# sunzeyeah/item-alignment

Measured on AMD Instinct MI355X. Metric: item-pairs/sec (train step) RoBERTa-large+ViT-B two-tower, higher is better.
Workload: dtype bf16

## Files before the change

include/itemalign.h:

```cpp
#ifndef ITEMALIGN_H
#define ITEMALIGN_H
#include <stddef.h>
#include <stdint.h>

#ifdef __cplusplus
extern "C" {
#endif

typedef struct ihipStream_t* ia_stream_t;

#define IA_OK 0
#define IA_ERR_ARG (-1)
#define IA_ERR_LAUNCH (-2)
#define IA_ERR_WORKSPACE (-3)
#define IA_ERR_UNSUPPORTED (-4)

const char* ia_strerror(int code);
#define IA_ABI_VERSION 20
int ia_abi_version(void);

#define IA_EPI_NONE 0
#define IA_EPI_BIAS 1
#define IA_EPI_BIAS_GELU 2
#define IA_EPI_ADD 3
// ... 10 lines not shown
size_t ia_gemm_colsum_workspace_bytes(int M, int N);
size_t ia_gemm_wgrad_rows_workspace_bytes(int N_out, int N_in, int M_rows);
int ia_gemm_wgrad_rows_filters(int N_out, int N_in, int M_rows);
int ia_gemm_wgrad_rows(const void* dY, int ldy, const void* X, int ldx, float* dW, int ldw, int N_out, int N_in, int M_rows,
                       const uint8_t* row_live, int accumulate, void* workspace, size_t workspace_bytes, ia_stream_t stream);
size_t ia_ktile_mask_bytes(int M_rows);
int ia_ktile_mask(const uint8_t* row_live, int M_rows, uint32_t* mask, ia_stream_t stream);
int ia_ktile_mask_host(const uint8_t* row_live, int M_rows, uint32_t* mask);
size_t ia_gemm_dgrad_rows_workspace_bytes(int M_rows, int N_in, int K_out);
int ia_gemm_dgrad_rows_filters(int M_rows, int N_in, int K_out);
int ia_gemm_dgrad_rows(const void* dY, int ldy, const void* W, int w_kstrided, int ldw, void* dX, int ldx, int M_rows, int N_in, int K_out,
                       int epilogue, const void* aux, int ldaux, void* C2, const uint8_t* row_live, void* workspace, size_t workspace_bytes,
                       ia_stream_t stream);
size_t ia_row_blocks_bytes(int M_rows);
int ia_row_blocks(const uint8_t* row_live, int M_rows, int* list, ia_stream_t stream);
int ia_row_blocks_host(const uint8_t* row_live, int M_rows, int* list);
int ia_debug_dgrad_rows(int on);
int ia_debug_fwd_rows(int on);
size_t ia_gemm_fwd_rows_workspace_bytes(int M_rows);
int ia_gemm_fwd_rows_filters(int M_rows, int N_out, int K_in);
int ia_gemm_fwd_rows(const void* X, int ldx, const void* W, int ldw, void* Y, int ldy, int M_rows, int N_out, int K_in, int epilogue,
                     const float* bias, void* C2, int scaled_cols, float col_scale, const uint8_t* row_live, int fill_dead_rows,
                     void* workspace, size_t workspace_bytes, ia_stream_t stream);
int ia_gemm_fwd_rows_add(const void* X, int ldx, const void* W, int ldw, void* Y, int ldy, int M_rows, int N_out, int K_in, const float* bias,
                         const void* aux, int ldaux, const uint8_t* row_live, int fill_dead_rows, void* workspace, size_t workspace_bytes,
                         ia_stream_t stream);
size_t ia_row_groups_bytes(int M_rows);
int ia_row_groups(const uint8_t* row_live, int M_rows, int* list, ia_stream_t stream);
int ia_row_groups_host(const uint8_t* row_live, int M_rows, int* list);
int ia_gemm_dgrad_groups_rows(const void* dY, int ldy, const void* W, int w_kstrided, int ldw, void* dX, int ldx, int M_rows, int N_in,
                              int K_out, const void* aux, int ldaux, void* C2, const uint8_t* row_live, void* workspace,
                              size_t workspace_bytes, ia_stream_t stream);
int ia_debug_out_rows(int on);

int ia_prof_begin(int variant, int max_launches);
int ia_prof_end(double* total_ms, double* total_flops, int* launches);
double ia_prof_bytes(void);
int ia_debug_cu_hog(int workgroups, float milliseconds, ia_stream_t stream);
int ia_debug_gemm_dynamic(int on);

int ia_ln_fwd(const void* x, const float* bias, const void* residual, void* z_out, void* y, float* mean, float* rstd,
              const float* gamma, const float* beta, int M, int H, float eps, float drop_p, uint32_t seed, uint32_t stream_id,
              ia_stream_t stream);
int ia_ln_fwd_rows(const void* x, const float* bias, const void* residual, void* z_out, void* y, float* mean, float* rstd,
                   const float* gamma, const float* beta, int M, int H, float eps, float drop_p, uint32_t seed, uint32_t stream_id,
                   const uint8_t* row_live, ia_stream_t stream);
size_t ia_ln_bwd_workspace_bytes(int M, int H);
int ia_ln_bwd(const void* dy, const void* dres, const void* z, const float* mean, const float* rstd, const float* gamma, void* dz,
              void* dx, float* dgamma, float* dbeta, float* dbias, int M, int H, float drop_p, uint32_t seed, uint32_t stream_id,
              void* workspace, size_t workspace_bytes, int accumulate, ia_stream_t stream);
int ia_ln_bwd2(const void* dy, const void* dy2, const void* dres, const void* z, const float* mean, const float* rstd, const float* gamma,
               void* dz, void* dx, float* dgamma, float* dbeta, float* dbias, int M, int H, float drop_p, uint32_t seed, uint32_t stream_id,
               void* workspace, size_t workspace_bytes, int accumulate, ia_stream_t stream);
int ia_ln_bwd2_rows(const void* dy, const void* dy2, const void* dres, const void* z, const float* mean, const float* rstd,
                    const float* gamma, void* dz, void* dx, float* dgamma, float* dbeta, float* dbias, int M, int H, float drop_p,
                    uint32_t seed, uint32_t stream_id, const uint8_t* row_live, void* workspace, size_t workspace_bytes, int accumulate,
                    ia_stream_t stream);
size_t ia_colsum_workspace_bytes(int M, int N);
int ia_colsum(const void* x, int ld, int M, int N, float* out, int accumulate, void* workspace, size_t workspace_bytes,
              ia_stream_t stream);

int ia_attn_fwd(const void* q, const void* k, const void* v, int ld_qkv, const uint8_t* key_mask, void* out, int ld_o, float* lse2,
                int B, int nh, int L, float scale, float drop_p, uint32_t seed, ia_stream_t stream);
int ia_attn_bwd(const void* q, const void* k, const void* v, int ld_qkv, const uint8_t* key_mask, const void* out, const void* d_out,
                int ld_o, const float* lse2, float* delta, void* dq, void* dk, void* dv, int ld_dqkv, int B, int nh, int L,
                float scale, float drop_p, uint32_t seed, ia_stream_t stream);
size_t ia_attn_bwd_bias_workspace_bytes(int B, int nh, int L);
int ia_attn_bwd_bias(const void* q, const void* k, const void* v, int ld_qkv, const uint8_t* key_mask, const void* out, const void* d_out,
                     int ld_o, const float* lse2, float* delta, void* dq, void* dk, void* dv, int ld_dqkv, float* dbias, void* workspace,
                     size_t workspace_bytes, int B, int nh, int L, float scale, float drop_p, uint32_t seed, ia_stream_t stream);

int ia_attn_fwd_ps(const void* q, const void* k, const void* v, int ld_qkv, const uint8_t* key_mask, void* out, int ld_o, float* lse2,
                   int B, int nh, int L, float scale, float drop_p, uint32_t seed, ia_stream_t stream);
int ia_attn_bwd_bias_ps(const void* q, const void* k, const void* v, int ld_qkv, const uint8_t* key_mask, const void* out, const void* d_out,
                        int ld_o, const float* lse2, float* delta, void* dq, void* dk, void* dv, int ld_dqkv, float* dbias, void* workspace,
                        size_t workspace_bytes, int B, int nh, int L, float scale, float drop_p, uint32_t seed, ia_stream_t stream);
#define IA_ATTN_Q_PRESCALED 1
#define IA_ATTN_MASKED_ROWS_DEAD 2
int ia_attn_bwd_bias_ex(int flags, const void* q, const void* k, const void* v, int ld_qkv, const uint8_t* key_mask, const void* out,
                        const void* d_out, int ld_o, const float* lse2, float* delta, void* dq, void* dk, void* dv, int ld_dqkv, float* dbias,
                        void* workspace, size_t workspace_bytes, int B, int nh, int L, float scale, float drop_p, uint32_t seed,
                        ia_stream_t stream);

int ia_attn_fwd_x(const void* q, int ld_q, const void* k, const void* v, int ld_kv, const uint8_t* key_mask, void* out, int ld_o,
                  float* lse2, int B, int nh, int Lq, int Lk, float scale, float drop_p, uint32_t seed, ia_stream_t stream);
int ia_attn_bwd_x(const void* q, int ld_q, const void* k, const void* v, int ld_kv, const uint8_t* key_mask, const void* out,
                  const void* d_out, int ld_o, const float* lse2, float* delta, void* dq, int ld_dq, void* dk, void* dv, int ld_dkv,
                  int B, int nh, int Lq, int Lk, float scale, float drop_p, uint32_t seed, ia_stream_t stream);
int ia_attn_fwd_causal_x(const void* q, int ld_q, const void* k, const void* v, int ld_kv, void* out, int ld_o, float* lse2, int B, int nh,
                         int Lk, int fold, float scale, ia_stream_t stream);
int ia_attn_bwd_causal_x(const void* q, int ld_q, const void* k, const void* v, int ld_kv, const void* out, const void* d_out, int ld_o,
                         const float* lse2, float* delta, void* dq, int ld_dq, void* dk, void* dv, int ld_dkv, int B, int nh, int Lk,
                         int fold, float scale, ia_stream_t stream);

int ia_rotary_split_fwd(const void* src, int ld_src, void* q_out, void* kv_out, int M, int n, int nh, ia_stream_t stream);
int ia_rotary_split_bwd(const void* dq, const void* dkv, void* dsrc, int ld_src, int M, int n, int nh, ia_stream_t stream);
int ia_swiglu_fwd(const void* src, int ld_src, void* out, int M, int F, ia_stream_t stream);
int ia_swiglu_bwd(const void* dout, const void* src, int ld_src, void* dsrc, int ld_dsrc, int M, int F, ia_stream_t stream);

int ia_kg_gather_fwd(const float* ent_table, const float* rel_table, const int64_t* ids, int ld_ids, int ent_col, int rel_lo,
                     float* h_sign, float* r, int B, int P, int Dk, ia_stream_t stream);
int ia_kg_gather_bwd(const float* dr, const int64_t* ids, int ld_ids, int rel_lo, float* rel_grad, int B, int P, int Dk,
                     ia_stream_t stream);
int ia_kg_rows_fwd(const float* h, const float* r, const float* hp, float* rows, int rows_per_item, int row0, int B, int P, int H,
                   ia_stream_t stream);
int ia_kg_rows_bwd(const float* drows, int rows_per_item, int row0, float* dh, float* dr, float* dhp, int B, int P, int H,
                   ia_stream_t stream);

#define IA_SIM_INNER 0
#define IA_SIM_COSINE 1
#define IA_SIM_L1 2
#define IA_SIM_L2 3
int ia_pair_sim_fwd(const float* x, const float* y, float* sim, float* probs, int B, int D, int measure, ia_stream_t stream);
int ia_pair_sim_bwd(const float* x, const float* y, const float* sim, const float* probs, const float* dsim, const float* dprobs,
                    float* dx, float* dy, int B, int D, int measure, ia_stream_t stream);
// ... 162 lines not shown
typedef struct {
  const void* w_qkv;
  const float* b_qkv;
  const void* w_o;
  const float* b_o;
  const float* ln1_g;
  const float* ln1_b;
  const void* w_fc1;
  const float* b_fc1;
  const void* w_fc2;
  const float* b_fc2;
  const float* ln2_g;
  const float* ln2_b;
  const void* wt_qkv;
  const void* wt_o;
  const void* wt_fc1;
  const void* wt_fc2;
} ia_layer_weights;

typedef struct {
  float* w_qkv; float* b_qkv; float* w_o; float* b_o; float* ln1_g; float* ln1_b;
  float* w_fc1; float* b_fc1; float* w_fc2; float* b_fc2; float* ln2_g; float* ln2_b;
} ia_layer_grads;

typedef struct {
  int B, L, H, I, nh;
  int pre_ln;
  float eps;
  float hidden_drop, attn_drop;
  uint32_t seed;
  uint32_t layer_id;
  const int* cu_seqlens;
  int total_tokens;
  float* dx_colsum_out;
  int dy_colsum_done;
  int masked_rows_dead;
  const int* row_blocks;
  const uint32_t* live_ktiles;
  const uint8_t* out_row_live;
  const int* out_row_blocks;
  const uint32_t* out_live_ktiles;
  const int* out_row_groups;
} ia_layer_cfg;

size_t ia_layer_stash_bytes(const ia_layer_cfg* cfg);
size_t ia_layer_bwd_scratch_bytes(const ia_layer_cfg* cfg);
int ia_layer_fwd(const ia_layer_cfg* cfg, const ia_layer_weights* w, const void* x, const uint8_t* key_mask, void* y, void* stash,
                 ia_stream_t stream);
size_t ia_layer_infer_scratch_bytes(const ia_layer_cfg* cfg);
int ia_layer_fwd_infer(const ia_layer_cfg* cfg, const ia_layer_weights* w, const void* x, const uint8_t* key_mask, void* y, void* scratch,
                       size_t scratch_bytes, ia_stream_t stream);
int ia_layer_bwd(const ia_layer_cfg* cfg, const ia_layer_weights* w, const ia_layer_grads* g, const void* x, const uint8_t* key_mask,
                 const void* y, const void* stash, const void* dy, void* dx, void* scratch, size_t scratch_bytes, ia_stream_t stream);
int ia_layer_bwd2(const ia_layer_cfg* cfg, const ia_layer_weights* w, const ia_layer_grads* g, const void* x, const uint8_t* key_mask,
                  const void* y, const void* stash, const void* dy, const void* dy2, void* dx, void* dx2, void* scratch,
                  size_t scratch_bytes, ia_stream_t stream);

#define IA_GCN_LONG_ROW 512
#define IA_GCN_SLAB_ROWS 1024
int ia_gcn_propagate_fwd(const int64_t* rowptr, const void* col, int col_is_64, const float* val, const float* x, const float* x0,
                         float* h, int N, int C, float alpha, float drop_p, uint32_t seed, uint32_t stream_id,
                         const int32_t* long_rows, int n_long, ia_stream_t stream);
int ia_gcn_propagate_bwd(const int64_t* rowptr_t, const void* col_t, int col_is_64, const float* val_t, const float* dh, float* dx,
                         float* dx0, int dx0_accumulate, int N, int C, float alpha, float drop_p, uint32_t seed, uint32_t stream_id,
                         const int32_t* long_rows_t, int n_long_t, ia_stream_t stream);
int ia_gcn_mix_fwd(const float* h, const float* W, float* out, int N, int C, float beta, float drop_p, uint32_t seed, uint32_t stream_id,
// ... 39 lines not shown
```

item_alignment_amd/_lib.py:

```python
import ctypes as C
import os

_HERE = os.path.dirname(os.path.abspath(__file__))
LIB_PATH = os.path.join(_HERE, "libitemalign_hip.so")

vp, i32, u32, f32, sz = C.c_void_p, C.c_int, C.c_uint32, C.c_float, C.c_size_t
PP, IP = C.POINTER(C.c_void_p), C.POINTER(C.c_int)


class LayerWeights(C.Structure):
    _fields_ = [(n, vp) for n in ("w_qkv", "b_qkv", "w_o", "b_o", "ln1_g", "ln1_b", "w_fc1", "b_fc1", "w_fc2", "b_fc2",
                                  "ln2_g", "ln2_b", "wt_qkv", "wt_o", "wt_fc1", "wt_fc2")]


class LayerGrads(C.Structure):
    _fields_ = [(n, vp) for n in ("w_qkv", "b_qkv", "w_o", "b_o", "ln1_g", "ln1_b", "w_fc1", "b_fc1", "w_fc2", "b_fc2",
                                  "ln2_g", "ln2_b")]


class LayerCfg(C.Structure):
    _fields_ = [("B", i32), ("L", i32), ("H", i32), ("I", i32), ("nh", i32), ("pre_ln", i32), ("eps", f32),
                ("hidden_drop", f32), ("attn_drop", f32), ("seed", u32), ("layer_id", u32), ("cu_seqlens", vp), ("total_tokens", i32),
                ("dx_colsum_out", vp), ("dy_colsum_done", i32), ("masked_rows_dead", i32),
                ("row_blocks", vp), ("live_ktiles", vp),
                ("out_row_live", vp), ("out_row_blocks", vp), ("out_live_ktiles", vp), ("out_row_groups", vp)]


SIGNATURES = {
    "ia_strerror": (C.c_char_p, [i32]),
    "ia_abi_version": (i32, []),
    "ia_gemm_bf16": (i32, [vp, i32, i32, vp, i32, i32, vp, i32, i32, i32, i32, i32, i32, vp, vp, i32, vp, i32, vp, sz, vp]),
    "ia_gemm_workspace_bytes": (sz, [i32, i32, i32, i32]),
    "ia_gemm_colsum_workspace_bytes": (sz, [i32, i32]),
    "ia_gemm_wgrad_rows_workspace_bytes": (sz, [i32, i32, i32]),
    "ia_gemm_wgrad_rows_filters": (i32, [i32, i32, i32]),
    "ia_gemm_wgrad_rows": (i32, [vp, i32, vp, i32, vp, i32, i32, i32, i32, vp, i32, vp, sz, vp]),
    "ia_ktile_mask_bytes": (sz, [i32]),
    "ia_ktile_mask": (i32, [vp, i32, vp, vp]),
    "ia_ktile_mask_host": (i32, [vp, i32, vp]),
    "ia_gemm_dgrad_rows_workspace_bytes": (sz, [i32, i32, i32]),
    "ia_gemm_dgrad_rows_filters": (i32, [i32, i32, i32]),
    "ia_gemm_dgrad_rows": (i32, [vp, i32, vp, i32, i32, vp, i32, i32, i32, i32, i32, vp, i32, vp, vp, vp, sz, vp]),
    "ia_row_blocks_bytes": (sz, [i32]),
    "ia_row_blocks": (i32, [vp, i32, vp, vp]),
    "ia_row_blocks_host": (i32, [vp, i32, vp]),
    "ia_debug_dgrad_rows": (i32, [i32]),
    "ia_gemm_fwd_rows_workspace_bytes": (sz, [i32]),
    "ia_gemm_fwd_rows_filters": (i32, [i32, i32, i32]),
    "ia_gemm_fwd_rows": (i32, [vp, i32, vp, i32, vp, i32, i32, i32, i32, i32, vp, vp, i32, f32, vp, i32, vp, sz, vp]),
    "ia_debug_fwd_rows": (i32, [i32]),
    "ia_gemm_fwd_rows_add": (i32, [vp, i32, vp, i32, vp, i32, i32, i32, i32, vp, vp, i32, vp, i32, vp, sz, vp]),
    "ia_row_groups_bytes": (sz, [i32]),
    "ia_row_groups": (i32, [vp, i32, vp, vp]),
    "ia_row_groups_host": (i32, [vp, i32, vp]),
    "ia_gemm_dgrad_groups_rows": (i32, [vp, i32, vp, i32, i32, vp, i32, i32, i32, i32, vp, i32, vp, vp, vp, sz, vp]),
    "ia_debug_out_rows": (i32, [i32]),
    "ia_prof_begin": (i32, [i32, i32]),
    "ia_prof_end": (i32, [C.POINTER(C.c_double), C.POINTER(C.c_double), C.POINTER(i32)]),
    "ia_prof_bytes": (C.c_double, []),
    "ia_debug_cu_hog": (i32, [i32, C.c_float, vp]),
    "ia_debug_gemm_dynamic": (i32, [i32]),
    "ia_ln_fwd": (i32, [vp, vp, vp, vp, vp, vp, vp, vp, vp, i32, i32, f32, f32, u32, u32, vp]),
    "ia_ln_fwd_rows": (i32, [vp, vp, vp, vp, vp, vp, vp, vp, vp, i32, i32, f32, f32, u32, u32, vp, vp]),
    "ia_ln_bwd_workspace_bytes": (sz, [i32, i32]),
    "ia_ln_bwd": (i32, [vp, vp, vp, vp, vp, vp, vp, vp, vp, vp, vp, i32, i32, f32, u32, u32, vp, sz, i32, vp]),
    "ia_ln_bwd2": (i32, [vp, vp, vp, vp, vp, vp, vp, vp, vp, vp, vp, vp, i32, i32, f32, u32, u32, vp, sz, i32, vp]),
    "ia_ln_bwd2_rows": (i32, [vp, vp, vp, vp, vp, vp, vp, vp, vp, vp, vp, vp, i32, i32, f32, u32, u32, vp, vp, sz, i32, vp]),
    "ia_colsum_workspace_bytes": (sz, [i32, i32]),
    "ia_colsum": (i32, [vp, i32, i32, i32, vp, i32, vp, sz, vp]),
    "ia_attn_fwd": (i32, [vp, vp, vp, i32, vp, vp, i32, vp, i32, i32, i32, f32, f32, u32, vp]),
    "ia_attn_bwd": (i32, [vp, vp, vp, i32, vp, vp, vp, i32, vp, vp, vp, vp, vp, i32, i32, i32, i32, f32, f32, u32, vp]),
    "ia_attn_bwd_bias_workspace_bytes": (sz, [i32, i32, i32]),
    "ia_attn_bwd_bias": (i32, [vp, vp, vp, i32, vp, vp, vp, i32, vp, vp, vp, vp, vp, i32, vp, vp, sz, i32, i32, i32, f32, f32, u32, vp]),
    "ia_attn_fwd_ps": (i32, [vp, vp, vp, i32, vp, vp, i32, vp, i32, i32, i32, f32, f32, u32, vp]),
    "ia_attn_bwd_bias_ps": (i32, [vp, vp, vp, i32, vp, vp, vp, i32, vp, vp, vp, vp, vp, i32, vp, vp, sz, i32, i32, i32, f32, f32, u32, vp]),
    "ia_attn_bwd_bias_ex": (i32, [i32, vp, vp, vp, i32, vp, vp, vp, i32, vp, vp, vp, vp, vp, i32, vp, vp, sz, i32, i32, i32, f32, f32, u32, vp]),
    "ia_gemm_bf16_qscale": (i32, [vp, i32, vp, i32, vp, i32, i32, i32, i32, vp, i32, f32, vp]),
    "ia_attn_fwd_x": (i32, [vp, i32, vp, vp, i32, vp, vp, i32, vp, i32, i32, i32, i32, f32, f32, u32, vp]),
    "ia_attn_bwd_x": (i32, [vp, i32, vp, vp, i32, vp, vp, vp, i32, vp, vp, vp, i32, vp, vp, i32, i32, i32, i32, i32, f32, f32, u32, vp]),
    "ia_attn_fwd_causal_x": (i32, [vp, i32, vp, vp, i32, vp, i32, vp, i32, i32, i32, i32, f32, vp]),
    "ia_attn_bwd_causal_x": (i32, [vp, i32, vp, vp, i32, vp, vp, i32, vp, vp, vp, i32, vp, vp, i32, i32, i32, i32, i32, f32, vp]),
    "ia_rotary_split_fwd": (i32, [vp, i32, vp, vp, i32, i32, i32, vp]),
    "ia_rotary_split_bwd": (i32, [vp, vp, vp, i32, i32, i32, i32, vp]),
    "ia_swiglu_fwd": (i32, [vp, i32, vp, i32, i32, vp]),
    "ia_swiglu_bwd": (i32, [vp, vp, i32, vp, i32, i32, i32, vp]),
    "ia_kg_gather_fwd": (i32, [vp, vp, vp, i32, i32, i32, vp, vp, i32, i32, i32, vp]),
    "ia_kg_gather_bwd": (i32, [vp, vp, i32, i32, vp, i32, i32, i32, vp]),
    "ia_kg_rows_fwd": (i32, [vp, vp, vp, vp, i32, i32, i32, i32, i32, vp]),
    "ia_kg_rows_bwd": (i32, [vp, i32, i32, vp, vp, vp, i32, i32, i32, vp]),
    "ia_pair_sim_fwd": (i32, [vp, vp, vp, vp, i32, i32, i32, vp]),
    "ia_pair_sim_bwd": (i32, [vp, vp, vp, vp, vp, vp, vp, vp, i32, i32, i32, vp]),
    "ia_nchw_to_nhwc_bf16": (i32, [vp, vp, i32, i32, i32, i32, i32, vp]),
    "ia_conv_nhwc_workspace_bytes": (sz, [i32, i32, i32, i32, i32, i32, i32, i32]),
    "ia_conv_nhwc_fwd": (i32, [vp, vp, vp, vp, i32, i32, i32, i32, i32, i32, i32, i32, vp, sz, vp]),
    "ia_conv_nhwc_bwd_data": (i32, [vp, vp, vp, i32, i32, i32, i32, i32, i32, i32, i32, vp, sz, vp]),
    "ia_conv_nhwc_bwd_weight": (i32, [vp, vp, vp, vp, i32, i32, i32, i32, i32, i32, i32, i32, i32, vp, sz, vp]),
    "ia_ws_conv_weight_fwd": (i32, [vp, vp, vp, vp, vp, i32, i32, i32, i32, f32, f32, vp]),
    "ia_ws_conv_weight_bwd": (i32, [vp, vp, vp, vp, vp, vp, vp, i32, i32, i32, i32, f32, vp]),
    "ia_silu_fwd": (i32, [vp, vp, sz, f32, vp]),
    "ia_silu_bwd": (i32, [vp, vp, vp, vp, sz, f32, vp]),
    "ia_silu_bwd_sum": (i32, [vp, vp, vp, vp, vp, sz, f32, vp]),
    "ia_avgpool2_fwd": (i32, [vp, vp, i32, i32, i32, i32, vp]),
    "ia_avgpool2_bwd": (i32, [vp, vp, i32, i32, i32, i32, vp]),
    "ia_gap_workspace_bytes": (sz, [i32, i32, i32]),
    "ia_gap_fwd": (i32, [vp, vp, i32, i32, i32, vp, sz, vp]),
    "ia_gap_bwd": (i32, [vp, vp, i32, i32, i32, vp]),
    "ia_eca_fwd": (i32, [vp, vp, i32, vp, vp, vp, vp, i32, i32, i32, f32, vp, sz, vp]),
    "ia_eca_fwd_linear_workspace_bytes": (sz, [i32, i32, i32]),
    "ia_eca_fwd_linear": (i32, [vp, vp, vp, vp, i32, vp, i32, vp, vp, vp, f32, vp, vp, i32, i32, i32, f32, vp, sz, vp]),
# ... 140 lines not shown
```

item_alignment_amd/csrc/attention.hip:

```cpp
#include "common.h"
#include <type_traits>
#include <cstdlib>

#define IA_ATTN_Q_PRESCALED 1
#define IA_ATTN_MASKED_ROWS_DEAD 2
extern "C" size_t ia_attn_bwd_bias_workspace_bytes(int B, int nh, int L);

namespace {

constexpr uint32_t OOB = 0xFFFFFFF0u;
constexpr float LOG2E = 1.4426950408889634f;

struct AttnArgs {
  const bf16* q; const bf16* k; const bf16* v;
  const bf16* o; const bf16* d_o;
  bf16* out;
  bf16* dq; bf16* dk; bf16* dv;
  const uint8_t* mask;
  float* lse2;
  float* delta;
  int B, nh, Lq, Lk;
  const int* cu;
  int ld_q, ld_kv, ld_o, ld_dq, ld_dkv;
  uint32_t q_bytes, kv_bytes, o_bytes;
  float sc;
  float scale;
  int q_prescaled;
  uint32_t thr16; float inv_keep; uint32_t seed;
  float* cs_part;
  int exact_delta;
  int dead_queries;
};

IA_DEV void attn_block_coords(const AttnArgs& p, int nt, int& tile, int& h, int& b) {
  const int nwg = gridDim.x, bid = blockIdx.x;
  const int per = nwg >> 3, r = nwg & 7, xcd = bid & 7, idx = bid >> 3;
  int w = (xcd < r ? xcd * (per + 1) : r * (per + 1) + (xcd - r) * per) + idx;
  tile = w % nt; w /= nt;
  h = w % p.nh; b = w / p.nh;
}

constexpr int MAX_KT = 32;
IA_DEV void build_valid_table(const AttnArgs& p, uint32_t (*s_valid)[2], size_t rowbase, int L, int lane, int wave) {
  const int nkt = (L + 63) >> 6;
  for (int t = wave; t < nkt; t += 4) {
    const int key = t * 64 + lane;
    const bool kv = key < L && (p.mask == nullptr || p.mask[rowbase + key] != 0);
    const uint64_t vb = __ballot(kv);
    if (lane == 0) { s_valid[t][0] = (uint32_t)vb; s_valid[t][1] = (uint32_t)(vb >> 32); }
  }
}

IA_DEV int swz_b128(int row) { return (row >> 1) & 7; }
IA_DEV int swz_tr(int row) { return ((row >> 1) & 1) << 2; }

IA_DEV void stage_rows32(__amdgpu_buffer_rsrc_t rs, char* slot, size_t row0, int nvalid, int ld, int col0, int lane) {
#pragma unroll
  for (int i = 0; i < 4; ++i) {
    const int row = i * 8 + (lane >> 3);
    const int c = (lane & 7) ^ swz_b128(row);
    uint32_t off = (uint32_t)(((row0 + row) * ld + col0 + c * 8) * 2);
    if (row >= nvalid) off = OOB;
    __builtin_amdgcn_raw_ptr_buffer_load_lds(rs, IA_LDS(slot + i * 1024), 16, off, 0, 0, 0);
  }
// ... 53 lines not shown
    *reinterpret_cast<bf16x4*>(w + 64 + rg * 16) = c;
  }
  asm volatile("s_waitcnt lgkmcnt(0)" ::: "memory");
  float cs[8];
#pragma unroll
  for (int j = 0; j < 8; ++j) cs[j] = 0.f;
#pragma unroll
  for (int i = 0; i < 4; ++i) {
    const int row = i * 8 + (lane >> 3), c = lane & 7;
    const bf16x8 v = *reinterpret_cast<const bf16x8*>(slot + row * EPI_ROW + c * 16);
    if (row < nrows) {
      *reinterpret_cast<bf16x8*>(out + (size_t)row * ld + c * 8) = v;
      if (cs_out) {
#pragma unroll
        for (int j = 0; j < 8; ++j) cs[j] += bf2f(v[j]);
      }
    }
  }
  if (cs_out) {
#pragma unroll
    for (int j = 0; j < 8; ++j) {
      float x = cs[j];
      x += ia_dpp<0x128>(x);
      cs[j] = ia_add_xor32(ia_add_xor16(x));
    }
    if (lane < 8) {
      *reinterpret_cast<f32x4*>(cs_out + lane * 8) = f32x4{cs[0], cs[1], cs[2], cs[3]};
      *reinterpret_cast<f32x4*>(cs_out + lane * 8 + 4) = f32x4{cs[4], cs[5], cs[6], cs[7]};
    }
  }
}
IA_DEV void zero_cs_row(float* cs_out, int lane) {
  if (lane < 16) *reinterpret_cast<f32x4*>(cs_out + lane * 4) = f32x4{0.f, 0.f, 0.f, 0.f};
}

namespace fwd3 {
constexpr int k_slot(int s) { return s == 2 ? 32768 : s * 8192; }
constexpr int v_slot(int s) { return s == 2 ? 40960 : 16384 + s * 8192; }
constexpr int Q_OFF = 32768, EPI_OFF = 0, TAB_OFF = 49152, SMEM = TAB_OFF + MAX_KT * 8;
constexpr uint32_t L_LO_BITS = 0x0D800000u, L_HI_BITS = 0x5D800000u;
constexpr float NEG_BIG = -1e30f;
constexpr uint32_t NEG_BIG_BF16 = 0xF14Au;

template <int OFF>
IA_DEV bf16x8 lds_read_b128(uint32_t addr) {
  bf16x8 d;
  asm volatile("ds_read_b128 %0, %1 offset:%2" : "=v"(d) : "v"(addr), "n"(OFF));
  return d;
}
template <int N>
IA_DEV void frag_wait(bf16x8 (&f)[8]) {
  asm volatile("s_waitcnt lgkmcnt(%8)" : "+v"(f[0]), "+v"(f[1]), "+v"(f[2]), "+v"(f[3]), "+v"(f[4]), "+v"(f[5]), "+v"(f[6]), "+v"(f[7]) : "n"(N));
}
IA_DEV float swap32(float x) {
  float a = x, b = x;
  asm volatile("s_nop 1\n\tv_permlane32_swap_b32 %0, %1\n\ts_nop 1" : "+v"(a), "+v"(b));
  return (threadIdx.x & 32) ? a : b;
}
IA_DEV f32x16 mfma(bf16x8 a, bf16x8 b, f32x16 c) { return __builtin_amdgcn_mfma_f32_32x32x16_bf16(a, b, c, 0, 0, 0); }

struct Lane {
  uint32_t ka[4];
  uint32_t v0, v1;
  uint32_t dk0, dk1, dv0, dv1;
};

// ... 78 lines not shown
  row.l_run *= alpha;
#pragma unroll
  for (int r = 0; r < 16; ++r) {
    s[r] = __builtin_amdgcn_exp2f(s[r] - m_new);
    o0[r] *= alpha; o1[r] *= alpha;
  }
  if (other) {
#pragma unroll
    for (int r = 0; r < 16; ++r) (*other)[r] += shift;
  }
}
}

template <bool DROPOUT, int QB>
__global__ __launch_bounds__(256, QB == 1 ? 3 : 2) void attn_fwd3_kernel(AttnArgs p) {
  using namespace fwd3;
  constexpr int ROWS = 128 * QB;
  constexpr int QX_OFF = SMEM;
  __shared__ __attribute__((aligned(16))) char smem[SMEM + (QB - 1) * 16384];
  uint32_t (*s_valid)[2] = reinterpret_cast<uint32_t (*)[2]>(smem + TAB_OFF);
  const int tid = threadIdx.x, lane = tid & 63, hh = lane >> 5, lq = lane & 31;
  const int wave = __builtin_amdgcn_readfirstlane(tid >> 6);
  int tile, h, b;
  attn_block_coords(p, (p.Lq + ROWS - 1) / ROWS, tile, h, b);
  int Lq = p.Lq, L = p.Lk;
  size_t qbase = (size_t)b * Lq, rowbase = (size_t)b * L;
  if (p.cu) {
    const int c0 = p.cu[b];
    Lq = L = p.cu[b + 1] - c0;
    qbase = rowbase = (size_t)c0;
    if (tile * ROWS >= Lq) return;
  }
  const int q0 = tile * ROWS + wave * 32 * QB;
  const bool active = q0 < Lq;
  const uint32_t win = (uint32_t)(((size_t)(L - 1) * p.ld_kv + 64) * 2);
  const __amdgpu_buffer_rsrc_t rsK = ia_rsrc(p.k + rowbase * p.ld_kv + h * 64, win);
  const __amdgpu_buffer_rsrc_t rsV = ia_rsrc(p.v + rowbase * p.ld_kv + h * 64, win);
  const uint32_t sbase = lds_addr(smem);
  const uint32_t tile_bytes = (uint32_t)p.ld_kv * 128u;
  const int nkt_all = (L + 63) >> 6;

  Lane ln;
  {
    const uint32_t a0 = (uint32_t)(lq * 128 + ((hh ^ swz_b128(lq)) << 4));
#pragma unroll
    for (int kb = 0; kb < 4; ++kb) ln.ka[kb] = sbase + (a0 ^ (uint32_t)(kb << 5));
    ln.v0 = sbase + tr_lane_off(lane, 0); ln.v1 = sbase + tr_lane_off(lane, 32);
    const int r0 = tid >> 3, r1 = 32 + (tid >> 3), c = tid & 7;
    ln.dk0 = (uint32_t)((r0 * p.ld_kv + (c ^ swz_b128(r0)) * 8) * 2); ln.dk1 = (uint32_t)((r1 * p.ld_kv + (c ^ swz_b128(r1)) * 8) * 2);
    ln.dv0 = (uint32_t)((r0 * p.ld_kv + (c ^ swz_tr(r0)) * 8) * 2);   ln.dv1 = (uint32_t)((r1 * p.ld_kv + (c ^ swz_tr(r1)) * 8) * 2);
  }
  typedef __attribute__((address_space(3))) char lds_char;
  lds_char* const lsm = (lds_char*)IA_LDS(smem);
  auto stage_k = [&](auto SLOT_T, int kt) {
    constexpr int S = decltype(SLOT_T)::value;
    const uint32_t so = (uint32_t)kt * tile_bytes;
    __builtin_amdgcn_raw_ptr_buffer_load_lds(rsK, (lsm + k_slot(S) + wave * 1024), 16, ln.dk0, so, 0, 0);
    __builtin_amdgcn_raw_ptr_buffer_load_lds(rsK, (lsm + k_slot(S) + 4096 + wave * 1024), 16, ln.dk1, so, 0, 0);
  };
  auto stage_v = [&](auto SLOT_T, int kt) {
    constexpr int S = decltype(SLOT_T)::value;
    const uint32_t so = (uint32_t)kt * tile_bytes;
    __builtin_amdgcn_raw_ptr_buffer_load_lds(rsV, (lsm + v_slot(S) + wave * 1024), 16, ln.dv0, so, 0, 0);
    __builtin_amdgcn_raw_ptr_buffer_load_lds(rsV, (lsm + v_slot(S) + 4096 + wave * 1024), 16, ln.dv1, so, 0, 0);
  };
  using S0 = std::integral_constant<int, 0>; using S1 = std::integral_constant<int, 1>; using S2 = std::integral_constant<int, 2>;

// ... 236 lines not shown
  for (int kb = 0; kb < 4; ++kb) {
    const bf16x8 raw = frag_b128(rq, lq, kb * 2 + hh);
    gf[kb] = frag_b128(rg, lq, kb * 2 + hh);
    const bf16x8 ov = frag_b128(ro, lq, kb * 2 + hh);
#pragma unroll
    for (int j = 0; j < 8; ++j) {
      dlt += bf2f(ov[j]) * bf2f(gf[kb][j]);
      qf[kb][j] = !p.q_prescaled ? f2bf(bf2f(raw[j]) * p.sc) : raw[j];
    }
  }
  dlt += swap32(dlt);
  if (p.exact_delta) dlt = p.delta[sidx];
  else if (active && hh == 0 && q < Lq) p.delta[sidx] = dlt;
  f32x16 nl, nd;
#pragma unroll
  for (int r = 0; r < 16; ++r) { nl[r] = -lse; nd[r] = DROPOUT ? 0.f : -dlt; }
  asm volatile("s_waitcnt lgkmcnt(0)" ::: "memory");
  __builtin_amdgcn_s_barrier();
  int nkt = nkt_all;
  uint32_t ragged = 0u;
  for (int t = 0; t < nkt_all; ++t) {
    const uint32_t lo = s_valid[t][0], hi = s_valid[t][1];
    if ((lo & hi) != 0xFFFFFFFFu) ragged |= 1u << t;
    if ((lo | hi) != 0u) nkt = t + 1;
  }
  bool work = active;
  if (p.dead_queries && p.cu == nullptr && p.Lq == p.Lk) {
    const uint32_t mine = active ? s_valid[q0 >> 6][(q0 >> 5) & 1] : 0u;
    const int t128 = tile * 2;
    uint32_t any = s_valid[t128][0] | s_valid[t128][1];
    if (t128 + 1 < nkt_all) any |= s_valid[t128 + 1][0] | s_valid[t128 + 1][1];
    work = active && __builtin_amdgcn_readfirstlane(mine) != 0u;
    if (__builtin_amdgcn_readfirstlane(any) == 0u) nkt = 1;
  }
  nkt = __builtin_amdgcn_readfirstlane(nkt);
  ragged = __builtin_amdgcn_readfirstlane(ragged);
  if (nkt > 1) stage_tile(S1{}, 1);
  const uint32_t rk = DROPOUT ? ia_rng_row(p.seed, (uint32_t)(b * p.nh + h), (uint32_t)q) : 0u;
  const uint32_t thr1 = DROPOUT ? (p.thr16 - 1u) * 0x10001u : 0u;
  f32x16 dq0 = zero16(), dq1 = zero16();

  auto tile_step = [&](auto SLOT_T, int t) {
    constexpr int SB = decltype(SLOT_T)::value * STAGE;
    using NEXT2 = std::integral_constant<int, (decltype(SLOT_T)::value + 2) % 3>;
    const bool LAST = t + 1 >= nkt;
    if (LAST) asm volatile("s_waitcnt vmcnt(0)" ::: "memory");
    else asm volatile("s_waitcnt vmcnt(4)" ::: "memory");
    __builtin_amdgcn_s_barrier();
    if (t + 2 < nkt) stage_tile(NEXT2{}, t + 2);
    if (!work) return;
    bf16x8 xk0, xk1, xv0, xv1, yk0, yk1, yv0, yv1;
    auto rd = [&](auto KB, bf16x8& k0, bf16x8& k1, bf16x8& v0, bf16x8& v1) {
      constexpr int kb = decltype(KB)::value;
      k0 = lds_read_b128<SB>(ka[kb]); k1 = lds_read_b128<SB + 4096>(ka[kb]);
      v0 = lds_read_b128<SB + 8192>(ka[kb]); v1 = lds_read_b128<SB + 12288>(ka[kb]);
    };
    using I0 = std::integral_constant<int, 0>; using I1 = std::integral_constant<int, 1>;
    using I2 = std::integral_constant<int, 2>; using I3 = std::integral_constant<int, 3>;
    rd(I0{}, xk0, xk1, xv0, xv1);
    rd(I1{}, yk0, yk1, yv0, yv1);
    f32x16 s0, s1, dp0, dp1;
    const bool plain = !((ragged >> t) & 1u);
    frag_wait4<4>(xk0, xk1, xv0, xv1);
    s0 = mfma(xk0, qf[0], nl); s1 = mfma(xk1, qf[0], nl);
    dp0 = mfma(xv0, gf[0], nd); dp1 = mfma(xv1, gf[0], nd);
    if (!plain) {
// ... 313 lines not shown
#pragma unroll
    for (int j = 0; j < 8; ++j) { kf[kb][j] = f2bf(-bf2f(kr[j])); vf[kb][j] = f2bf(-bf2f(vr[j])); }
  }
  const bool scale_q = !p.q_prescaled;
  if (scale_q) {
#pragma unroll
    for (int i = 0; i < 2; ++i) {
      bf16x8* const qp = reinterpret_cast<bf16x8*>(smem + i * 4096 + wave * 1024 + lane * 16);
      bf16x8 v = *qp;
#pragma unroll
      for (int j = 0; j < 8; ++j) v[j] = f2bf(bf2f(v[j]) * p.sc);
      *qp = v;
    }
  }
  int* const s_last = reinterpret_cast<int*>(smem + 3 * KV_STAGE + 1024 + 512);
  const bool trim = p.dead_queries && p.mask != nullptr && p.cu == nullptr && p.Lq == p.Lk;
  if (trim) {
    int last = -1;
    for (int base = wave * 64; base < Lq; base += 256) {
      const int pos = base + lane;
      const bool ok = pos < Lq && p.mask[rowbase + pos] != 0;
      const uint64_t bal = __ballot(ok);
      if (bal) last = base + 63 - __builtin_clzll(bal);
    }
    if (lane == 0) s_last[wave] = last;
  }
  asm volatile("s_waitcnt lgkmcnt(0)" ::: "memory");
  __builtin_amdgcn_s_barrier();
  if (trim) {
    const int last = max(max(s_last[0], s_last[1]), max(s_last[2], s_last[3]));
    const int live = __builtin_amdgcn_readfirstlane(last < 0 ? 1 : (last >> 6) + 1);
    if (live < nqt) nqt = live;
  }
  if (nqt > 1) stage_tile(S1{}, 1);
  f32x16 dk0 = zero16(), dk1 = zero16(), dv0 = zero16(), dv1 = zero16();

  auto prescale = [&](int stage_base) {
#pragma unroll
    for (int i = 0; i < 2; ++i) {
      bf16x8* const qp = reinterpret_cast<bf16x8*>(smem + stage_base + i * 4096 + wave * 1024 + lane * 16);
      bf16x8 v = *qp;
#pragma unroll
      for (int j = 0; j < 8; ++j) v[j] = f2bf(bf2f(v[j]) * sc);
      *qp = v;
    }
  };
  auto tile_step = [&](auto SLOT_T, int qt) {
    constexpr int SB = decltype(SLOT_T)::value * KV_STAGE;
    using NEXT2 = std::integral_constant<int, (decltype(SLOT_T)::value + 2) % 3>;
    if (qt + 1 >= nqt) asm volatile("s_waitcnt vmcnt(0)" ::: "memory");
    else asm volatile("s_waitcnt vmcnt(5)" ::: "memory");
    asm volatile("s_waitcnt lgkmcnt(0)" ::: "memory");
    __builtin_amdgcn_s_barrier();
    if (qt + 2 < nqt) stage_tile(NEXT2{}, qt + 2);
    if (!active) {
      if (scale_q && qt + 1 < nqt) {
        if (qt + 2 < nqt) asm volatile("s_waitcnt vmcnt(5)" ::: "memory");
        else asm volatile("s_waitcnt vmcnt(0)" ::: "memory");
        prescale(((decltype(SLOT_T)::value + 1) % 3) * KV_STAGE);
      }
      return;
    }
    if (DROPOUT) {
      s_rk[lane] = ia_rng_row(seed, stream_id, (uint32_t)(qt * 64 + lane));
      __builtin_amdgcn_wave_barrier();
    }
// ... 36 lines not shown
        for (int rg = 0; rg < 4; ++rg) rkq[rg] = *(const lds_u32x4*)(s_rk + qs * 32 + 8 * rg + 4 * hh);
      }
#pragma unroll
      for (int r = 0; r < 16; ++r) {
        const float pv = __builtin_amdgcn_exp2f(-s[r]);
        float pd = pv, nds;
        if (DROPOUT) {
          const uint32_t hsh = ia_rng_pair(rkq[r >> 2][r & 3], pc);
          const uint32_t dr = (hsh >> ush) & 0xFFFFu;
          const float mk = __builtin_fminf(__builtin_fmaxf((float)((int)dr - (int)thr1), 0.f), 1.f);
          pd = pv * mk;
          nds = pv * __builtin_fmaf(dp[r] * mk, inv_keep, dlr[r]);
        } else {
          nds = pv * dp[r];
        }
        pf[r >> 3][r & 7] = f2bf(pd);
        sf[r >> 3][r & 7] = f2bf(nds);
      }
      tr_wait<12>(g0);
      dv0 = mfma(g0.a0(), pf[0], dv0); dv1 = mfma(g0.a1(), pf[0], dv1);
      tr_wait<8>(a0);
      dk0 = mfma(a0.a0(), sf[0], dk0); dk1 = mfma(a0.a1(), sf[0], dk1);
      tr_wait<4>(g1);
      dv0 = mfma(g1.a0(), pf[1], dv0); dv1 = mfma(g1.a1(), pf[1], dv1);
      tr_wait<0>(a1);
      dk0 = mfma(a1.a0(), sf[1], dk0); dk1 = mfma(a1.a1(), sf[1], dk1);
    };
    sub_tile(std::integral_constant<int, 0>{});
    if (scale_q && qt + 1 < nqt) {
      if (qt + 2 < nqt) asm volatile("s_waitcnt vmcnt(5)" ::: "memory");
      else asm volatile("s_waitcnt vmcnt(0)" ::: "memory");
      prescale(((decltype(SLOT_T)::value + 1) % 3) * KV_STAGE);
    }
    if (qt * 64 + 32 < Lq) sub_tile(std::integral_constant<int, 1>{});
  };
  {
    int qt = 0;
    for (;;) {
      tile_step(S0{}, qt); if (++qt >= nqt) break;
      tile_step(S1{}, qt); if (++qt >= nqt) break;
      tile_step(S2{}, qt); if (++qt >= nqt) break;
    }
  }
  __builtin_amdgcn_s_barrier();
  float* cs_lds = p.cs_part ? reinterpret_cast<float*>(smem + 8 * EPI_SLOT) + wave * 128 : nullptr;
  if (!active && !cs_lds) return;
  if (active) {
    store_block_rows(smem + wave * 2 * EPI_SLOT, dk0, dk1, -1.f / LOG2E, !key_ok, p.dk + (rowbase + k0) * p.ld_dkv + h * 64, p.ld_dkv,
                     L - k0, lane, cs_lds);
    store_block_rows(smem + (wave * 2 + 1) * EPI_SLOT, dv0, dv1, DROPOUT ? p.inv_keep : 1.f, !key_ok, p.dv + (rowbase + k0) * p.ld_dkv + h * 64,
                     p.ld_dkv, L - k0, lane, cs_lds ? cs_lds + 64 : nullptr);
  } else { zero_cs_row(cs_lds, lane); zero_cs_row(cs_lds + 64, lane); }
  if (cs_lds) {
    __syncthreads();
    if (wave < 2) {
      const float* c = reinterpret_cast<const float*>(smem + 8 * EPI_SLOT) + wave * 64;
      p.cs_part[(size_t)(b * ((p.Lk + 127) >> 7) + tile) * (3 * p.nh * 64) + (1 + wave) * p.nh * 64 + h * 64 + lane] =
          (c[lane] + c[128 + lane]) + (c[256 + lane] + c[384 + lane]);
    }
  }
}

namespace bwdf {
using namespace bwd3;
constexpr int NW = 8, RING = 4;
constexpr int SL_Q = 0, SL_G = 4096, SL_O = 8192, SL_LSE = 12288, SL_DLT = SL_LSE + 256, SL_RK = SL_LSE + 384, SLOT = SL_LSE + 512;
constexpr int DLT_F = (SL_DLT - SL_LSE) / 4;
// ... 113 lines not shown
      for (int i = 0; i < 8; ++i) d += bf2f(gv[i]) * bf2f(ov[i]);
      d += ia_dpp<0xB1>(d); d += ia_dpp<0x4E>(d); d += ia_dpp<0x141>(d);
      if (c8 == 0) *reinterpret_cast<float*>(sl + SL_DLT + ((wave - 4) * 8 + r8) * 4) = d;
    }
  };

  const uint32_t thr1 = DROPOUT ? p.thr16 - 1u : 0u;
  const float inv_keep = p.inv_keep;
  const int ntile = (L + 127) >> 7;

  Cur prod{first_item, first_item / nh, first_item % nh};
  Cur cons = prod, kvn = prod;
  int pj = 0;
  issue_kv(kvn); adv(kvn);
#pragma unroll 1
  for (int s = 0; s < RING; ++s) {
    issue_ring(prod, pj, s);
    if (++pj == nb) { pj = 0; adv(prod); }
  }
  asm volatile("s_waitcnt vmcnt(0)" ::: "memory");
  prep(cons.it, 0, 0);
  asm volatile("s_waitcnt lgkmcnt(0)" ::: "memory");
  __builtin_amdgcn_s_barrier();

  bf16x8 kf[4], vf[4], KT[8];
  f32x16 dk0, dk1, dv0, dv1;
  f32x4 csq;
  bool key_ok = false, mine = false;
  uint32_t vbits = 0u;
  float pen = 0.f;
  bool any_bad = false;
  uint32_t pc = 0u, ush = 0u;
  const int G = cnt * nb;
  int cj = 0;
  Cur prev = cons;
  int pcj = 0;
#pragma unroll 1
  for (int g = 0;; ++g) {
    const bool haveA = g < G;
    const bool first = cj == 0, last = cj == nb - 1;
    auto part_a = [&](int ga, bool first_a, int blk) {
      {
        const int slot = ga & (RING - 1), par = ga & 1;
        if (first_a) {
          const char* kb_ = smem + KST + wave * 4096;
          const char* vb_ = smem + VST + wave * 4096;
#pragma unroll
          for (int kb = 0; kb < 4; ++kb) {
            const bf16x8 kr = frag_u(kb_, lk, kb * 2 + hh), vr = frag_u(vb_, lk, kb * 2 + hh);
#pragma unroll
            for (int i = 0; i < 8; ++i) { kf[kb][i] = f2bf(-bf2f(kr[i])); vf[kb][i] = f2bf(-bf2f(vr[i])); }
          }
          {
            s16x4 lo[8], hi[8];
#pragma unroll
            for (int k = 0; k < 8; ++k) { lo[k] = tr_read<0>(ktb + k * 4096); hi[k] = tr_read<2048>(ktb + k * 4096); }
            asm volatile("s_waitcnt lgkmcnt(0)" : "+v"(lo[0]), "+v"(lo[1]), "+v"(lo[2]), "+v"(lo[3]), "+v"(lo[4]), "+v"(lo[5]), "+v"(lo[6]), "+v"(lo[7]));
            asm volatile("" : "+v"(hi[0]), "+v"(hi[1]), "+v"(hi[2]), "+v"(hi[3]), "+v"(hi[4]), "+v"(hi[5]), "+v"(hi[6]), "+v"(hi[7]));
#pragma unroll
            for (int k = 0; k < 8; ++k) KT[k] = join(lo[k], hi[k]);
          }
          const int key = wave * 32 + lk;
          {
            const uint32_t* const mw = reinterpret_cast<const uint32_t*>(smem + MSK_OFF);
            uint32_t vb = 0u;
#pragma unroll
            for (int k = 0; k < 8; ++k) vb |= (mw[k] != 0u ? 1u : 0u) << k;
            vbits = __builtin_amdgcn_readfirstlane(vb);
            key_ok = ((mw[wave] >> lk) & 1u) != 0u;
          }
          mine = ((vbits >> wave) & 1u) != 0u;
          pen = key_ok ? 0.f : PEN;
          any_bad = __ballot(!key_ok) != 0ull;
          pc = pair_c_of(key); ush = (uint32_t)(key & 1) * 16u;
          dk0 = zero16(); dk1 = zero16(); dv0 = zero16(); dv1 = zero16();
          csq = f32x4{0.f, 0.f, 0.f, 0.f};
        }
        if (mine && (!p.dead_queries || ((vbits >> blk) & 1u))) {
          const uint32_t so = (uint32_t)(slot * SLOT);
          f32x16 s, dp;
          const float* const sL = reinterpret_cast<const float*>(smem + RING_OFF + slot * SLOT + SL_LSE) + 4 * hh;
          {
#pragma unroll
            for (int rg = 0; rg < 4; ++rg) {
              const f32x4 ls = *reinterpret_cast<const f32x4*>(sL + 8 * rg);
              const f32x4 dl = *reinterpret_cast<const f32x4*>(sL + DLT_F + 8 * rg);
#pragma unroll
              for (int j = 0; j < 4; ++j) { s[rg * 4 + j] = ls[j]; dp[rg * 4 + j] = DROPOUT ? 0.f : dl[j]; }
            }
            if (any_bad) {
#pragma unroll
              for (int r = 0; r < 16; ++r) s[r] += pen;
            }
          }
          const uint32_t k0_ = ka0 + so;
          bf16x8 xq, xg, yq, yg;
          xq = lds_read_b128<SL_Q>(k0_); xg = lds_read_b128<SL_G>(k0_);
          yq = lds_read_b128<SL_Q>(k0_ ^ 32u); yg = lds_read_b128<SL_G>(k0_ ^ 32u);
          asm volatile("s_waitcnt lgkmcnt(2)" : "+v"(xq), "+v"(xg));
          s = mfma(xq, kf[0], s); dp = mfma(xg, vf[0], dp);
          xq = lds_read_b128<SL_Q>(k0_ ^ 64u); xg = lds_read_b128<SL_G>(k0_ ^ 64u);
          asm volatile("s_waitcnt lgkmcnt(2)" : "+v"(yq), "+v"(yg));
          s = mfma(yq, kf[1], s); dp = mfma(yg, vf[1], dp);
          yq = lds_read_b128<SL_Q>(k0_ ^ 96u); yg = lds_read_b128<SL_G>(k0_ ^ 96u);
          asm volatile("s_waitcnt lgkmcnt(2)" : "+v"(xq), "+v"(xg));
          s = mfma(xq, kf[2], s); dp = mfma(xg, vf[2], dp);
          const uint32_t a0_ = t0 + so, a1_ = a0_ + t1d, a0x = a0_ ^ 32u, a1x = a1_ ^ 32u;
          TrPair g0, q0, g1, q1;
          read_tr<SL_G, 0>(g0, a0_, a1_, a0x, a1x);
          read_tr<SL_Q, 0>(q0, a0_, a1_, a0x, a1x);
          asm volatile("s_waitcnt lgkmcnt(8)" : "+v"(yq), "+v"(yg));
// ... 19 lines not shown
              pf[hf][rr] = f2bf(pd);
              sf[hf][rr] = f2bf(nds);
            }
            const int xa = xwo + par * XT;
            *reinterpret_cast<bf16x4*>(smem + (xa ^ (hf * 32))) = bf16x4{sf[hf][0], sf[hf][1], sf[hf][2], sf[hf][3]};
            *reinterpret_cast<bf16x4*>(smem + (xa ^ (hf * 32 + 16))) = bf16x4{sf[hf][4], sf[hf][5], sf[hf][6], sf[hf][7]};
          };
          half(std::integral_constant<int, 0>{});
          read_tr<SL_G, 16>(g1, a0_, a1_, a0x, a1x);
          read_tr<SL_Q, 16>(q1, a0_, a1_, a0x, a1x);
          tr_wait<12>(g0);
          dv0 = mfma(g0.a0(), pf[0], dv0); dv1 = mfma(g0.a1(), pf[0], dv1);
          tr_wait<8>(q0);
          dk0 = mfma(q0.a0(), sf[0], dk0); dk1 = mfma(q0.a1(), sf[0], dk1);
          half(std::integral_constant<int, 1>{});
          tr_wait<4>(g1);
          dv0 = mfma(g1.a0(), pf[1], dv0); dv1 = mfma(g1.a1(), pf[1], dv1);
          tr_wait<0>(q1);
          dk0 = mfma(q1.a0(), sf[1], dk0); dk1 = mfma(q1.a1(), sf[1], dk1);
        }
      }
    };
    auto part_c = [&]() {
      if (haveA && g >= 1) {
        if (cj == 1) { issue_kv(kvn); adv(kvn); }
        issue_ring(prod, pj, (g - 1) & (RING - 1));
        if (++pj == nb) { pj = 0; adv(prod); }
      }
      if (g == 0) return;
      {
        const uint32_t xr = xrb + ((g - 1) & 1) * XT, xr2 = xr ^ 16u;
        s16x4 lo[8], hi[8];
        f32x4 acc = {0.f, 0.f, 0.f, 0.f};
        if (!p.dead_queries || ((vbits >> pcj) & 1u)) {
#pragma unroll
        for (int k = 0; k < 8; ++k) { lo[k] = tr_read<0>(xr + k * 2 * XT); hi[k] = tr_read<16 * XP>(xr2 + k * 2 * XT); }
#define IA_DQ_STEP(k, n)                                                                                   \
        wait2<n>(lo[k], hi[k]);                                                                            \
        if ((vbits >> k) & 1u) acc = mfma16(KT[k], join(lo[k], hi[k]), acc);
        IA_DQ_STEP(0, 14) IA_DQ_STEP(1, 12) IA_DQ_STEP(2, 10) IA_DQ_STEP(3, 8) IA_DQ_STEP(4, 6) IA_DQ_STEP(5, 4) IA_DQ_STEP(6, 2) IA_DQ_STEP(7, 0)
#undef IA_DQ_STEP
        }
        const int q = pcj * 32 + 16 * qh + p16;
        bf16x4 o4;
#pragma unroll
        for (int i = 0; i < 4; ++i) { o4[i] = f2bf(-p.scale * acc[i]); }
        if (q < L) {
          *reinterpret_cast<bf16x4*>(p.dq + ((size_t)prev.b * L + q) * p.ld_dq + prev.h * 64 + 16 * dqt + 4 * g4) = o4;
#pragma unroll
          for (int i = 0; i < 4; ++i) csq[i] += bf2f(o4[i]);
        }
      }
      if (!first) return;
      asm volatile("s_waitcnt lgkmcnt(0)" ::: "memory");
      __builtin_amdgcn_s_barrier();
      const size_t row0 = (size_t)prev.b * L;
      float* const cs_w = reinterpret_cast<float*>(smem + CS_OFF) + wave * 128;
      if (wave < nb) {
        store_block_rows(smem + X_OFF + wave * EPI_SLOT, dk0, dk1, -1.f / LOG2E, false, p.dk + (row0 + wave * 32) * p.ld_dkv + prev.h * 64, p.ld_dkv,
                         L - wave * 32, lane, p.cs_part ? cs_w : nullptr);
        store_block_rows(smem + X_OFF + wave * EPI_SLOT, dv0, dv1, DROPOUT ? inv_keep : 1.f, false, p.dv + (row0 + wave * 32) * p.ld_dkv + prev.h * 64,
                         p.ld_dkv, L - wave * 32, lane, p.cs_part ? cs_w + 64 : nullptr);
      } else if (p.cs_part) { zero_cs_row(cs_w, lane); zero_cs_row(cs_w + 64, lane); }
      if (p.cs_part) {
        int ln = lane;
        asm volatile("" : "+v"(ln));
        float* const cq = reinterpret_cast<float*>(smem + CS_OFF + NW * 128 * 4);
// ... 67 lines not shown
  a.inv_keep = drop_p > 0.f ? 1.f / (1.f - (float)a.thr16 / 65536.f) : 1.f;
  a.seed = seed;
  return IA_OK;
}

bool exact_delta_on() { const char* e = getenv("IA_ATTN_EXACT_DELTA"); return e && atoi(e) != 0; }
bool fused_applies(const AttnArgs& a) {
  return !a.exact_delta && a.cu == nullptr && a.Lq == a.Lk && a.Lq > 32 && a.Lq <= 256 && a.delta != nullptr;
}
template <bool D> void launch_fused(const AttnArgs& a, hipStream_t st) {
  hipLaunchKernelGGL(attn_key_bits_kernel, dim3(a.B), dim3(64), 0, st, a.mask, reinterpret_cast<uint32_t*>(a.delta), a.Lk);
  const int per_x = (a.B * a.nh + 7) / 8;
  const dim3 grid(8 * (per_x < 32 ? per_x : 32));
  hipLaunchKernelGGL(attn_bwd_fused_kernel<D>, grid, dim3(512), 0, st, a);
}
template <bool D> void launch_pair(const AttnArgs& a, hipStream_t st) {
  const dim3 gq(((a.Lq + 127) / 128) * a.nh * a.B), gk(((a.Lk + 127) / 128) * a.nh * a.B), blk(256);
  if (a.exact_delta) hipLaunchKernelGGL(attn_bwd3_delta_kernel<D>, gq, blk, 0, st, a);
  hipLaunchKernelGGL(attn_bwd3_dq_kernel<D>, gq, blk, 0, st, a);
  hipLaunchKernelGGL(attn_bwd3_dkv_kernel<D>, gk, blk, 0, st, a);
}
template <bool D> void launch_bwd(const AttnArgs& a, hipStream_t st) {
  if (fused_applies(a)) launch_fused<D>(a, st);
  else launch_pair<D>(a, st);
}
template <bool D> void launch_fwd(const AttnArgs& a, hipStream_t st) {
  if (((a.Lq - 1) & 255) < 128) hipLaunchKernelGGL((attn_fwd3_kernel<D, 1>), dim3(((a.Lq + 127) / 128) * a.nh * a.B), dim3(256), 0, st, a);
  else hipLaunchKernelGGL((attn_fwd3_kernel<D, 2>), dim3(((a.Lq + 255) / 256) * a.nh * a.B), dim3(256), 0, st, a);
}

struct Packed { const int* cu; int total; };
struct BiasOut { float* dbias; void* workspace; size_t workspace_bytes; };

int attn_fwd_impl(int flags, const void* q, int ld_q, const void* k, const void* v, int ld_kv, const uint8_t* key_mask, const Packed* pk, void* out,
                  int ld_o, float* lse2, int B, int nh, int Lq, int Lk, float scale, float drop_p, uint32_t seed, hipStream_t stream) {
  (void)hipGetLastError();
  if (!q || !k || !v || !out || (pk && (!pk->cu || pk->total <= 0))) return IA_ERR_ARG;
  AttnArgs a{};
  const int rc = fill_args(a, B, nh, Lq, Lk, ld_q, ld_kv, ld_o, scale, drop_p, seed, pk ? pk->total : 0);
  if (rc) return rc;
  a.q = (const bf16*)q; a.k = (const bf16*)k; a.v = (const bf16*)v; a.out = (bf16*)out; a.mask = key_mask; a.lse2 = lse2;
  a.cu = pk ? pk->cu : nullptr;
  a.q_prescaled = (flags & IA_ATTN_Q_PRESCALED) ? 1 : 0;
  if (a.thr16) launch_fwd<true>(a, stream);
  else launch_fwd<false>(a, stream);
  return ia_check_launch();
}

int attn_bwd_impl(int flags, const void* q, int ld_q, const void* k, const void* v, int ld_kv, const uint8_t* key_mask, const Packed* pk,
                  const void* out, const void* d_out, int ld_o, const float* lse2, float* delta, void* dq, int ld_dq, void* dk, void* dv, int ld_dkv,
                  const BiasOut* bias, int B, int nh, int Lq, int Lk, float scale, float drop_p, uint32_t seed, hipStream_t stream) {
  (void)hipGetLastError();
  if (!q || !k || !v || !out || !d_out || !lse2 || !delta || !dq || !dk || !dv) return IA_ERR_ARG;
  if ((pk && (!pk->cu || pk->total <= 0)) || (bias && !bias->dbias)) return IA_ERR_ARG;
  if (bias && (!bias->workspace || bias->workspace_bytes < ia_attn_bwd_bias_workspace_bytes(B, nh, Lq))) return IA_ERR_WORKSPACE;
  AttnArgs a{};
  int rc = fill_args(a, B, nh, Lq, Lk, ld_q, ld_kv, ld_o, scale, drop_p, seed, pk ? pk->total : 0);
  if (rc) return rc;
  if ((ld_dq & 7) || (ld_dkv & 7) || ld_dq < nh * 64 || ld_dkv < nh * 64) return IA_ERR_ARG;
  a.q = (const bf16*)q; a.k = (const bf16*)k; a.v = (const bf16*)v; a.o = (const bf16*)out; a.d_o = (const bf16*)d_out;
  a.mask = key_mask; a.lse2 = const_cast<float*>(lse2); a.delta = delta; a.cu = pk ? pk->cu : nullptr;
  a.dq = (bf16*)dq; a.dk = (bf16*)dk; a.dv = (bf16*)dv; a.ld_dq = ld_dq; a.ld_dkv = ld_dkv;
  a.cs_part = bias ? (float*)bias->workspace : nullptr;
  a.q_prescaled = (flags & IA_ATTN_Q_PRESCALED) ? 1 : 0;
  a.dead_queries = ((flags & IA_ATTN_MASKED_ROWS_DEAD) && key_mask) ? 1 : 0;
  a.exact_delta = exact_delta_on() ? 1 : 0;
  if (a.thr16) launch_bwd<true>(a, stream);
  else launch_bwd<false>(a, stream);
  rc = ia_check_launch();
  if (rc || !bias) return rc;
  return ia_sum_rows_f32((const float*)bias->workspace, B * ((Lq + 127) / 128), 3 * nh * 64, bias->dbias, 1, stream);
}

}

extern "C" int ia_attn_fwd_x(const void* q, int ld_q, const void* k, const void* v, int ld_kv, const uint8_t* key_mask, void* out,
                             int ld_o, float* lse2, int B, int nh, int Lq, int Lk, float scale, float drop_p, uint32_t seed,
                             hipStream_t stream) {
  return attn_fwd_impl(0, q, ld_q, k, v, ld_kv, key_mask, nullptr, out, ld_o, lse2, B, nh, Lq, Lk, scale, drop_p, seed, stream);
}

extern "C" int ia_attn_bwd_x(const void* q, int ld_q, const void* k, const void* v, int ld_kv, const uint8_t* key_mask,
                             const void* out, const void* d_out, int ld_o, const float* lse2, float* delta, void* dq, int ld_dq,
                             void* dk, void* dv, int ld_dkv, int B, int nh, int Lq, int Lk, float scale, float drop_p, uint32_t seed,
                             hipStream_t stream) {
  return attn_bwd_impl(0, q, ld_q, k, v, ld_kv, key_mask, nullptr, out, d_out, ld_o, lse2, delta, dq, ld_dq, dk, dv, ld_dkv, nullptr, B, nh, Lq, Lk,
                       scale, drop_p, seed, stream);
}

extern "C" int ia_attn_fwd(const void* q, const void* k, const void* v, int ld_qkv, const uint8_t* key_mask, void* out,
                           int ld_o, float* lse2, int B, int nh, int L, float scale, float drop_p, uint32_t seed,
                           hipStream_t stream) {
  return attn_fwd_impl(0, q, ld_qkv, k, v, ld_qkv, key_mask, nullptr, out, ld_o, lse2, B, nh, L, L, scale, drop_p, seed, stream);
}

extern "C" int ia_attn_fwd_ps(const void* q, const void* k, const void* v, int ld_qkv, const uint8_t* key_mask, void* out, int ld_o,
                              float* lse2, int B, int nh, int L, float scale, float drop_p, uint32_t seed, hipStream_t stream) {
  return attn_fwd_impl(IA_ATTN_Q_PRESCALED, q, ld_qkv, k, v, ld_qkv, key_mask, nullptr, out, ld_o, lse2, B, nh, L, L, scale, drop_p, seed, stream);
}

extern "C" int ia_attn_bwd(const void* q, const void* k, const void* v, int ld_qkv, const uint8_t* key_mask, const void* out,
                           const void* d_out, int ld_o, const float* lse2, float* delta, void* dq, void* dk, void* dv,
                           int ld_dqkv, int B, int nh, int L, float scale, float drop_p, uint32_t seed, hipStream_t stream) {
  return attn_bwd_impl(0, q, ld_qkv, k, v, ld_qkv, key_mask, nullptr, out, d_out, ld_o, lse2, delta, dq, ld_dqkv, dk, dv, ld_dqkv, nullptr, B, nh, L, L,
                       scale, drop_p, seed, stream);
}

extern "C" size_t ia_attn_bwd_bias_workspace_bytes(int B, int nh, int L) {
  if (B <= 0 || nh <= 0 || L <= 0) return 0;
  return (size_t)B * ((L + 127) / 128) * 3 * nh * 64 * sizeof(float);
}

extern "C" int ia_attn_bwd_bias_ex(int flags, const void* q, const void* k, const void* v, int ld_qkv, const uint8_t* key_mask, const void* out,
                                   const void* d_out, int ld_o, const float* lse2, float* delta, void* dq, void* dk, void* dv, int ld_dqkv,
                                   float* dbias, void* workspace, size_t workspace_bytes, int B, int nh, int L, float scale, float drop_p,
                                   uint32_t seed, hipStream_t stream) {
  if (flags & ~(IA_ATTN_Q_PRESCALED | IA_ATTN_MASKED_ROWS_DEAD)) return IA_ERR_ARG;
  const BiasOut bias{dbias, workspace, workspace_bytes};
  return attn_bwd_impl(flags, q, ld_qkv, k, v, ld_qkv, key_mask, nullptr, out, d_out, ld_o, lse2, delta, dq, ld_dqkv, dk, dv, ld_dqkv, &bias, B, nh, L, L,
                       scale, drop_p, seed, stream);
}
extern "C" int ia_attn_bwd_bias(const void* q, const void* k, const void* v, int ld_qkv, const uint8_t* key_mask, const void* out,
                                const void* d_out, int ld_o, const float* lse2, float* delta, void* dq, void* dk, void* dv, int ld_dqkv,
                                float* dbias, void* workspace, size_t workspace_bytes, int B, int nh, int L, float scale, float drop_p,
                                uint32_t seed, hipStream_t stream) {
  return ia_attn_bwd_bias_ex(0, q, k, v, ld_qkv, key_mask, out, d_out, ld_o, lse2, delta, dq, dk, dv, ld_dqkv, dbias, workspace, workspace_bytes, B, nh,
                             L, scale, drop_p, seed, stream);
}
extern "C" int ia_attn_bwd_bias_ps(const void* q, const void* k, const void* v, int ld_qkv, const uint8_t* key_mask, const void* out,
                                   const void* d_out, int ld_o, const float* lse2, float* delta, void* dq, void* dk, void* dv, int ld_dqkv,
                                   float* dbias, void* workspace, size_t workspace_bytes, int B, int nh, int L, float scale, float drop_p,
                                   uint32_t seed, hipStream_t stream) {
  return ia_attn_bwd_bias_ex(IA_ATTN_Q_PRESCALED, q, k, v, ld_qkv, key_mask, out, d_out, ld_o, lse2, delta, dq, dk, dv, ld_dqkv, dbias, workspace,
                             workspace_bytes, B, nh, L, scale, drop_p, seed, stream);
}

extern "C" int ia_attn_fwd_varlen(const void* q, const void* k, const void* v, int ld_qkv, const int* cu_seqlens, int total_tokens, void* out,
                                  int ld_o, float* lse2, int B, int nh, int Lmax, float scale, float drop_p, uint32_t seed, hipStream_t stream) {
  const Packed pk{cu_seqlens, total_tokens};
  return attn_fwd_impl(0, q, ld_qkv, k, v, ld_qkv, nullptr, &pk, out, ld_o, lse2, B, nh, Lmax, Lmax, scale, drop_p, seed, stream);
}
extern "C" int ia_attn_fwd_varlen_ps(const void* q, const void* k, const void* v, int ld_qkv, const int* cu_seqlens, int total_tokens, void* out,
                                     int ld_o, float* lse2, int B, int nh, int Lmax, float scale, float drop_p, uint32_t seed,
                                     hipStream_t stream) {
  const Packed pk{cu_seqlens, total_tokens};
  return attn_fwd_impl(IA_ATTN_Q_PRESCALED, q, ld_qkv, k, v, ld_qkv, nullptr, &pk, out, ld_o, lse2, B, nh, Lmax, Lmax, scale, drop_p, seed, stream);
}
extern "C" int ia_attn_bwd_varlen(const void* q, const void* k, const void* v, int ld_qkv, const int* cu_seqlens, int total_tokens,
                                  const void* out, const void* d_out, int ld_o, const float* lse2, float* delta, void* dq, void* dk, void* dv,
                                  int ld_dqkv, int B, int nh, int Lmax, float scale, float drop_p, uint32_t seed, hipStream_t stream) {
  const Packed pk{cu_seqlens, total_tokens};
  return attn_bwd_impl(0, q, ld_qkv, k, v, ld_qkv, nullptr, &pk, out, d_out, ld_o, lse2, delta, dq, ld_dqkv, dk, dv, ld_dqkv, nullptr, B, nh, Lmax, Lmax,
                       scale, drop_p, seed, stream);
}
// ... 8 lines not shown
```

item_alignment_amd/csrc/engine.hip:

```cpp
#include "common.h"
#include "../../include/itemalign.h"

namespace {

inline size_t al(size_t b) { return (b + 255) & ~(size_t)255; }
inline size_t rows_of(const ia_layer_cfg* c) { return c->cu_seqlens ? (size_t)c->total_tokens : (size_t)c->B * c->L; }

struct Carver {
  char* base; size_t bytes = 0;
  char* take(size_t b) { char* r = base ? base + bytes : nullptr; bytes += al(b); return r; }
};

struct FwdBufs {
  char* qkv; char* ctx;
  char* xn;
  char* proj;
  char* ln;
  char* ffn;
  char* hpre;
  char* hact;
  float* lse; float* mean1; float* rstd1; float* mean2; float* rstd2;
  int* row_blk;
  int* out_blk;
  size_t bytes;
// ... 9 lines not shown
  Carver a{(char*)base};
  FwdBufs s;
  s.qkv = a.take(M * 3 * H * 2); s.ctx = a.take(M * H * 2);
  char* t0 = a.take(M * H * 2); char* t1 = a.take(M * H * 2); char* t2 = a.take(M * H * 2);
  name_rows(s, c->pre_ln, t0, t1, t2);
  s.hpre = a.take(M * I * 2); s.hact = a.take(M * I * 2);
  s.lse = (float*)a.take((size_t)c->B * c->nh * c->L * 4);
  s.mean1 = (float*)a.take(M * 4); s.rstd1 = (float*)a.take(M * 4);
  s.mean2 = (float*)a.take(M * 4); s.rstd2 = (float*)a.take(M * 4);
  s.row_blk = (int*)a.take(ia_row_blocks_bytes((int)M));
  s.out_blk = (int*)a.take(ia_row_blocks_bytes((int)M));
  s.bytes = a.bytes;
  return s;
}

FwdBufs carve_infer(const ia_layer_cfg* c, void* base) {
  const size_t M = rows_of(c), H = c->H, I = c->I;
  Carver a{(char*)base};
  FwdBufs s;
  s.qkv = a.take(M * 3 * H * 2); s.ctx = a.take(M * H * 2);
  char* t0 = a.take(M * H * 2); char* t1 = a.take(M * H * 2);
  name_rows(s, c->pre_ln, t0, t1, t0);
  s.hpre = nullptr; s.hact = a.take(M * I * 2);
  s.lse = (float*)a.take((size_t)c->B * c->nh * c->L * 4);
  s.mean1 = s.mean2 = (float*)a.take(M * 4); s.rstd1 = s.rstd2 = (float*)a.take(M * 4);
  s.row_blk = (int*)a.take(ia_row_blocks_bytes((int)M));
  s.out_blk = (int*)a.take(ia_row_blocks_bytes((int)M));
  s.bytes = a.bytes;
  return s;
}

struct Scratch {
  char* g0; char* g1; char* g2; char* gI; char* gqkv; float* delta; char* ws; size_t ws_bytes; char* gws; size_t gws_bytes; uint32_t* live_kt; int* row_blk;
  uint32_t* out_kt; int* out_blk; int* out_grp;
  size_t bytes;
};

size_t max3(size_t a, size_t b, size_t c) { return a > b ? (a > c ? a : c) : (b > c ? b : c); }

Scratch carve_scratch(const ia_layer_cfg* c, void* base) {
  const size_t M = rows_of(c), H = c->H, I = c->I;
  Carver a{(char*)base};
  Scratch s;
  s.g0 = a.take(M * H * 2); s.g1 = a.take(M * H * 2); s.g2 = a.take(M * H * 2);
  s.gI = a.take(M * I * 2); s.gqkv = a.take(M * 3 * H * 2);
  s.delta = (float*)a.take((size_t)c->B * c->nh * c->L * 4);
  s.ws_bytes = max3(ia_ln_bwd_workspace_bytes((int)M, (int)H), ia_gemm_colsum_workspace_bytes((int)M, (int)I),
                    max3(ia_colsum_workspace_bytes((int)M, (int)(3 * H)), ia_attn_bwd_bias_workspace_bytes(c->B, c->nh, c->L), 0));
  s.ws = a.take(s.ws_bytes);
  s.gws_bytes = max3(ia_gemm_workspace_bytes((int)(3 * H), (int)H, (int)M, 1), ia_gemm_workspace_bytes((int)I, (int)H, (int)M, 1),
                     max3(ia_gemm_workspace_bytes((int)H, (int)I, (int)M, 1), ia_gemm_workspace_bytes((int)H, (int)H, (int)M, 1), 0));
  s.gws = a.take(s.gws_bytes);
  s.live_kt = (uint32_t*)a.take(ia_ktile_mask_bytes((int)M));
  s.row_blk = (int*)a.take(ia_row_blocks_bytes((int)M));
  s.out_kt = (uint32_t*)a.take(ia_ktile_mask_bytes((int)M));
  s.out_blk = (int*)a.take(ia_row_blocks_bytes((int)M));
  s.out_grp = (int*)a.take(ia_row_groups_bytes((int)M));
  s.bytes = a.bytes;
  return s;
}

bool cfg_ok(const ia_layer_cfg* c) {
  if (c && c->cu_seqlens && (c->total_tokens <= 0 || c->total_tokens > c->B * c->L)) return false;
  return c && c->B > 0 && c->L > 0 && c->H > 0 && c->I > 0 && c->nh > 0 && c->H == c->nh * 64 && (c->H & 7) == 0 && (c->I & 7) == 0;
}

int g_dgrad_rows = 1;
int g_fwd_rows = 1;
int g_out_rows = 1;
const uint8_t* out_live(const ia_layer_cfg* c) { return (c->out_row_live && !c->cu_seqlens && g_out_rows) ? c->out_row_live : nullptr; }

#define IA_TRY(expr) do { int rc_ = (expr); if (rc_) return rc_; } while (0)

int dgrad(const void* dy, int k_out, const void* w, const void* wt, int n_in, void* dx, int M, int epilogue, const void* aux, int ldaux, void* c2,
          void* ws, size_t ws_bytes, ia_stream_t st, const int* row_blk = nullptr, const int* row_grp = nullptr) {
  if (row_grp && epilogue == IA_EPI_DGELU_COLSUM)
    return ia_gemm_dgrad_groups(dy, k_out, wt ? wt : w, wt ? 0 : 1, wt ? k_out : n_in, dx, n_in, M, n_in, k_out, aux, ldaux, c2, row_grp, ws, ws_bytes, st);
  if (row_blk)
    return ia_gemm_dgrad_blocks(dy, k_out, wt ? wt : w, wt ? 0 : 1, wt ? k_out : n_in, dx, n_in, M, n_in, k_out, epilogue, aux, ldaux, c2, row_blk,
                                ws, ws_bytes, st);
  if (wt)
    return ia_gemm_bf16(dy, 0, k_out, wt, 0, k_out, dx, 0, n_in, M, n_in, k_out, epilogue, nullptr, aux, ldaux, c2, 0, ws, ws_bytes, st);
  return ia_gemm_bf16(dy, 0, k_out, w, 1, n_in, dx, 0, n_in, M, n_in, k_out, epilogue, nullptr, aux, ldaux, c2, 0, ws, ws_bytes, st);
}

int wgrad(const void* dy, int n_out, const void* x, int n_in, float* dw, int M, const uint32_t* live_kt, void* ws, size_t ws_bytes, ia_stream_t st) {
  if (live_kt) return ia_gemm_wgrad_masked(dy, n_out, x, n_in, dw, n_in, n_out, n_in, M, live_kt, 1, ws, ws_bytes, st);
  return ia_gemm_bf16(dy, 1, n_out, x, 1, n_in, dw, 1, n_in, n_out, n_in, M, IA_EPI_NONE, nullptr, nullptr, 0, nullptr, 1, ws, ws_bytes, st);
}

bool q_prescale(const ia_layer_cfg* c) { return (c->H & 127) == 0; }
int qkv_proj(const ia_layer_cfg* c, const void* x, const ia_layer_weights* w, void* qkv, int M, float scale, ia_stream_t st,
             const int* row_blk = nullptr) {
  const int H = c->H;
  if (row_blk)
    return ia_gemm_fwd_blocks(x, H, w->w_qkv, H, qkv, 3 * H, M, 3 * H, H, IA_EPI_BIAS, w->b_qkv, nullptr, q_prescale(c) ? H : 0,
                              q_prescale(c) ? scale * 1.4426950408889634f : 1.f, row_blk, 1, st);
  if (q_prescale(c)) return ia_gemm_bf16_qscale(x, H, w->w_qkv, H, qkv, 3 * H, M, 3 * H, H, w->b_qkv, H, scale * 1.4426950408889634f, st);
  return ia_gemm_bf16(x, 0, H, w->w_qkv, 0, H, qkv, 0, 3 * H, M, 3 * H, H, IA_EPI_BIAS, w->b_qkv, nullptr, 0, nullptr, 0, nullptr, 0, st);
}

int attn_fwd(const ia_layer_cfg* c, const char* qkv, const uint8_t* key_mask, char* ctx, float* lse, float scale, float drop, uint32_t seed,
             ia_stream_t st) {
  const int H = c->H;
  const bool ps = q_prescale(c);
  if (c->cu_seqlens)
    return (ps ? ia_attn_fwd_varlen_ps : ia_attn_fwd_varlen)(qkv, qkv + (size_t)H * 2, qkv + (size_t)2 * H * 2, 3 * H, c->cu_seqlens, c->total_tokens, ctx, H, lse, c->B, c->nh,
                              c->L, scale, drop, seed, st);
  return (ps ? ia_attn_fwd_ps : ia_attn_fwd)(qkv, qkv + (size_t)H * 2, qkv + (size_t)2 * H * 2, 3 * H, key_mask, ctx, H, lse, c->B, c->nh, c->L, scale, drop, seed, st);
}

int attn_bwd(const ia_layer_cfg* c, const char* qkv, const uint8_t* key_mask, const char* ctx, const char* dctx, const float* lse, float* delta,
             char* gqkv, float* db_qkv, void* ws, size_t ws_bytes, float scale, float drop, uint32_t seed, ia_stream_t st) {
  const int H = c->H;
  const bool ps = q_prescale(c);
  if (c->cu_seqlens) {
    int rc = (ps ? ia_attn_bwd_varlen_ps : ia_attn_bwd_varlen)(qkv, qkv + (size_t)H * 2, qkv + (size_t)2 * H * 2, 3 * H, c->cu_seqlens, c->total_tokens, ctx, dctx, H, lse, delta,
                                gqkv, gqkv + (size_t)H * 2, gqkv + (size_t)2 * H * 2, 3 * H, c->B, c->nh, c->L, scale, drop, seed, st);
    return rc ? rc : ia_colsum(gqkv, 3 * H, (int)rows_of(c), 3 * H, db_qkv, 1, ws, ws_bytes, st);
  }
  const int flags = (ps ? IA_ATTN_Q_PRESCALED : 0) | ((c->masked_rows_dead & 1) ? IA_ATTN_MASKED_ROWS_DEAD : 0);
  return ia_attn_bwd_bias_ex(flags, qkv, qkv + (size_t)H * 2, qkv + (size_t)2 * H * 2, 3 * H, key_mask, ctx, dctx, H, lse, delta, gqkv,
                             gqkv + (size_t)H * 2, gqkv + (size_t)2 * H * 2, 3 * H, db_qkv, ws, ws_bytes, c->B, c->nh, c->L, scale, drop, seed, st);
}

int layer_forward(const ia_layer_cfg* c, const ia_layer_weights* w, const void* x, const uint8_t* key_mask, void* y, const FwdBufs& s,
                  bool keep, ia_stream_t st) {
  const int M = (int)rows_of(c), H = c->H, I = c->I;
  const float scale = 0.125f;
  const int gelu = keep ? IA_EPI_BIAS_GELU : IA_EPI_BIAS_GELU_ACT;
  if (!c->pre_ln) {
    const float hidden_drop = keep ? c->hidden_drop : 0.f, attn_drop = keep ? c->attn_drop : 0.f;
    const uint32_t seed = keep ? c->seed : 0u, attn_seed = keep ? c->seed * 2654435761u + c->layer_id * 97u + 17u : 0u;
    const uint32_t ln1_stream = keep ? c->layer_id * 4u + 0u : 0u, ln2_stream = keep ? c->layer_id * 4u + 1u : 0u;
    const uint8_t* live = ((c->masked_rows_dead & 3) == 3 && !c->cu_seqlens && key_mask && g_fwd_rows) ? key_mask : nullptr;
    const int* row_blk = nullptr;
    if (live) {
      row_blk = c->row_blocks;
      if (!row_blk) { IA_TRY(ia_row_blocks(live, M, s.row_blk, st)); row_blk = s.row_blk; }
    }
    IA_TRY(qkv_proj(c, x, w, s.qkv, M, scale, st, row_blk));
    IA_TRY(attn_fwd(c, s.qkv, key_mask, s.ctx, s.lse, scale, attn_drop, attn_seed, st));
    if (const uint8_t* const olive = out_live(c)) {
      live = olive;
      row_blk = c->out_row_blocks;
      if (!row_blk) { IA_TRY(ia_row_blocks(olive, M, s.out_blk, st)); row_blk = s.out_blk; }
    }
    if (row_blk) IA_TRY(ia_gemm_fwd_blocks(s.ctx, H, w->w_o, H, s.proj, H, M, H, H, IA_EPI_NONE, nullptr, nullptr, 0, 1.f, row_blk, 0, st));
    else IA_TRY(ia_gemm_bf16(s.ctx, 0, H, w->w_o, 0, H, s.proj, 0, H, M, H, H, IA_EPI_NONE, nullptr, nullptr, 0, nullptr, 0, nullptr, 0, st));
    IA_TRY(ia_ln_fwd_rows(s.proj, w->b_o, x, keep ? s.proj : nullptr, s.ln, s.mean1, s.rstd1, w->ln1_g, w->ln1_b, M, H, c->eps, hidden_drop, seed,
                          ln1_stream, live, st));
    if (row_blk) IA_TRY(ia_gemm_fwd_blocks(s.ln, H, w->w_fc1, H, s.hact, I, M, I, H, gelu, w->b_fc1, s.hpre, 0, 1.f, row_blk, 1, st));
    else IA_TRY(ia_gemm_bf16(s.ln, 0, H, w->w_fc1, 0, H, s.hact, 0, I, M, I, H, gelu, w->b_fc1, nullptr, 0, s.hpre, 0, nullptr, 0, st));
    if (row_blk) IA_TRY(ia_gemm_fwd_blocks(s.hact, I, w->w_fc2, I, s.ffn, H, M, H, I, IA_EPI_NONE, nullptr, nullptr, 0, 1.f, row_blk, 0, st));
    else IA_TRY(ia_gemm_bf16(s.hact, 0, I, w->w_fc2, 0, I, s.ffn, 0, H, M, H, I, IA_EPI_NONE, nullptr, nullptr, 0, nullptr, 0, nullptr, 0, st));
    IA_TRY(ia_ln_fwd_rows(s.ffn, w->b_fc2, s.ln, keep ? s.ffn : nullptr, y, s.mean2, s.rstd2, w->ln2_g, w->ln2_b, M, H, c->eps, hidden_drop, seed,
// ... 3 lines not shown
    IA_TRY(qkv_proj(c, s.xn, w, s.qkv, M, scale, st));
    IA_TRY(attn_fwd(c, s.qkv, key_mask, s.ctx, s.lse, scale, 0.f, 0, st));
    const uint8_t* const olive = out_live(c);
    const int* oblk = nullptr;
    if (olive) {
      oblk = c->out_row_blocks;
      if (!oblk) { IA_TRY(ia_row_blocks(olive, M, s.out_blk, st)); oblk = s.out_blk; }
    }
    if (oblk) IA_TRY(ia_gemm_fwd_blocks(s.ctx, H, w->w_o, H, s.proj, H, M, H, H, IA_EPI_NONE, nullptr, nullptr, 0, 1.f, oblk, 0, st));
    else IA_TRY(ia_gemm_bf16(s.ctx, 0, H, w->w_o, 0, H, s.proj, 0, H, M, H, H, IA_EPI_NONE, nullptr, nullptr, 0, nullptr, 0, nullptr, 0, st));
    IA_TRY(ia_ln_fwd_rows(s.proj, w->b_o, x, s.proj, s.ln, s.mean2, s.rstd2, w->ln2_g, w->ln2_b, M, H, c->eps, 0.f, 0, 0, olive, st));
    if (oblk) {
      IA_TRY(ia_gemm_fwd_blocks(s.ln, H, w->w_fc1, H, s.hact, I, M, I, H, gelu, w->b_fc1, s.hpre, 0, 1.f, oblk, 1, st));
      IA_TRY(ia_gemm_fwd_blocks_add(s.hact, I, w->w_fc2, I, y, H, M, H, I, w->b_fc2, s.proj, H, oblk, 0, st));
    } else {
      IA_TRY(ia_gemm_bf16(s.ln, 0, H, w->w_fc1, 0, H, s.hact, 0, I, M, I, H, gelu, w->b_fc1, nullptr, 0, s.hpre, 0, nullptr, 0, st));
      IA_TRY(ia_gemm_bf16(s.hact, 0, I, w->w_fc2, 0, I, y, 0, H, M, H, I, IA_EPI_BIAS_ADD, w->b_fc2, s.proj, H, nullptr, 0, nullptr, 0, st));
    }
  }
  return IA_OK;
}

}

extern "C" int ia_debug_fwd_rows(int on) {
  const int was = g_fwd_rows;
  g_fwd_rows = on ? 1 : 0;
  return was;
}

extern "C" int ia_debug_out_rows(int on) {
  const int was = g_out_rows;
  g_out_rows = on ? 1 : 0;
  return was;
}

extern "C" int ia_debug_dgrad_rows(int on) {
  const int was = g_dgrad_rows;
  g_dgrad_rows = on ? 1 : 0;
  return was;
}

extern "C" size_t ia_layer_stash_bytes(const ia_layer_cfg* cfg) {
  (void)hipGetLastError();
  if (!cfg_ok(cfg)) return 0;
  return carve_stash(cfg, nullptr).bytes;
}

extern "C" size_t ia_layer_bwd_scratch_bytes(const ia_layer_cfg* cfg) {
  (void)hipGetLastError();
  if (!cfg_ok(cfg)) return 0;
  return carve_scratch(cfg, nullptr).bytes;
}

extern "C" size_t ia_layer_infer_scratch_bytes(const ia_layer_cfg* cfg) {
  (void)hipGetLastError();
  if (!cfg_ok(cfg)) return 0;
  return carve_infer(cfg, nullptr).bytes;
}

extern "C" int ia_layer_fwd(const ia_layer_cfg* c, const ia_layer_weights* w, const void* x, const uint8_t* key_mask, void* y,
                            void* stash, ia_stream_t st) {
  (void)hipGetLastError();
  if (!cfg_ok(c) || !w || !x || !y || !stash) return IA_ERR_ARG;
  if (c->pre_ln && (c->hidden_drop > 0.f || c->attn_drop > 0.f)) return IA_ERR_UNSUPPORTED;
  return layer_forward(c, w, x, key_mask, y, carve_stash(c, stash), true, st);
// ... 15 lines not shown
                            const uint8_t* key_mask, const void* y, const void* stash, const void* dy, void* dx, void* scratch,
                            size_t scratch_bytes, ia_stream_t st) {
  return ia_layer_bwd2(c, w, g, x, key_mask, y, stash, dy, nullptr, dx, nullptr, scratch, scratch_bytes, st);
}

extern "C" int ia_layer_bwd2(const ia_layer_cfg* c, const ia_layer_weights* w, const ia_layer_grads* g, const void* x,
                             const uint8_t* key_mask, const void* y, const void* stash, const void* dy, const void* dy2, void* dx, void* dx2,
                             void* scratch, size_t scratch_bytes, ia_stream_t st) {
  (void)hipGetLastError();
  (void)y;
  if (!cfg_ok(c) || !w || !g || !x || !stash || !dy || !dx || !scratch) return IA_ERR_ARG;
  if (c->pre_ln && (dy2 || dx2)) return IA_ERR_UNSUPPORTED;
  if (scratch_bytes < ia_layer_bwd_scratch_bytes(c)) return IA_ERR_WORKSPACE;
  const int M = (int)rows_of(c), H = c->H, I = c->I;
  const FwdBufs s = carve_stash(c, const_cast<void*>(stash));
  const Scratch k = carve_scratch(c, scratch);
  const float scale = 0.125f;
  const uint32_t attn_seed = c->seed * 2654435761u + c->layer_id * 97u + 17u;
  const bool drop = c->hidden_drop > 0.f;
  const uint8_t* const olive = out_live(c);
  const uint32_t* okt = nullptr; const int* oblk = nullptr; const int* ogrp = nullptr;
  if (olive) {
    okt = c->out_live_ktiles; oblk = c->out_row_blocks; ogrp = c->out_row_groups;
    if (!okt) { IA_TRY(ia_ktile_mask(olive, M, k.out_kt, st)); okt = k.out_kt; }
    if (!oblk) { IA_TRY(ia_row_blocks(olive, M, k.out_blk, st)); oblk = k.out_blk; }
    if (!ogrp) { IA_TRY(ia_row_groups(olive, M, k.out_grp, st)); ogrp = k.out_grp; }
  }
  if (!c->pre_ln) {
    const uint8_t* const live = ((c->masked_rows_dead & 1) && !c->cu_seqlens) ? key_mask : nullptr;
    const uint32_t* const live_kt = live ? (c->live_ktiles ? c->live_ktiles : k.live_kt) : nullptr;
    const int* const row_blk = (live && g_dgrad_rows) ? (c->row_blocks ? c->row_blocks : k.row_blk) : nullptr;
    if (live && !c->live_ktiles) IA_TRY(ia_ktile_mask(live, M, k.live_kt, st));
    if (row_blk && !c->row_blocks) IA_TRY(ia_row_blocks(live, M, k.row_blk, st));
    const uint8_t* const live2 = olive ? olive : live;
    const uint32_t* const kt2 = olive ? okt : live_kt;
    const int* const blk2 = olive ? oblk : row_blk;
    IA_TRY(ia_ln_bwd2_rows(dy, dy2, nullptr, s.ffn, s.mean2, s.rstd2, w->ln2_g, k.g0, drop ? k.g1 : nullptr, g->ln2_g, g->ln2_b, g->b_fc2, M, H,
                           c->hidden_drop, c->seed, c->layer_id * 4u + 1u, live2, k.ws, k.ws_bytes, 1, st));
    const char* d_ffn = drop ? k.g1 : k.g0;
    IA_TRY(wgrad(d_ffn, H, s.hact, I, (float*)g->w_fc2, M, kt2, k.gws, k.gws_bytes, st));
    IA_TRY(dgrad(d_ffn, H, w->w_fc2, w->wt_fc2, I, k.gI, M, IA_EPI_DGELU_COLSUM, s.hpre, I, g->b_fc1, k.ws, k.ws_bytes, st, nullptr, ogrp));
    IA_TRY(wgrad(k.gI, I, s.ln, H, (float*)g->w_fc1, M, kt2, k.gws, k.gws_bytes, st));
    IA_TRY(dgrad(k.gI, I, w->w_fc1, w->wt_fc1, H, k.g2, M, IA_EPI_NONE, nullptr, 0, nullptr, nullptr, 0, st, blk2));
    char* dz1buf = dx2 ? (char*)dx2 : k.g0;
    IA_TRY(ia_ln_bwd2_rows(k.g2, k.g0, nullptr, s.proj, s.mean1, s.rstd1, w->ln1_g, dz1buf, drop ? k.g1 : nullptr, g->ln1_g, g->ln1_b, g->b_o, M, H,
                           c->hidden_drop, c->seed, c->layer_id * 4u + 0u, live2, k.ws, k.ws_bytes, 1, st));
    const char* d_att = drop ? k.g1 : dz1buf;
    IA_TRY(wgrad(d_att, H, s.ctx, H, (float*)g->w_o, M, kt2, k.gws, k.gws_bytes, st));
    IA_TRY(dgrad(d_att, H, w->w_o, w->wt_o, H, k.g2, M, IA_EPI_NONE, nullptr, 0, nullptr, nullptr, 0, st, blk2));
    IA_TRY(attn_bwd(c, s.qkv, key_mask, s.ctx, k.g2, s.lse, k.delta, k.gqkv, g->b_qkv, k.ws, k.ws_bytes, scale, c->attn_drop, attn_seed, st));
    IA_TRY(wgrad(k.gqkv, 3 * H, x, H, (float*)g->w_qkv, M, live_kt, k.gws, k.gws_bytes, st));
    if (dx2)
      IA_TRY(dgrad(k.gqkv, 3 * H, w->w_qkv, w->wt_qkv, H, dx, M, IA_EPI_NONE, nullptr, 0, nullptr, nullptr, 0, st, row_blk));
    else
      IA_TRY(dgrad(k.gqkv, 3 * H, w->w_qkv, w->wt_qkv, H, dx, M, IA_EPI_ADD, dz1buf, H, nullptr, nullptr, 0, st, row_blk));
  } else {
    if (!c->dy_colsum_done) IA_TRY(ia_colsum(dy, H, M, H, g->b_fc2, 1, k.ws, k.ws_bytes, st));
    IA_TRY(wgrad(dy, H, s.hact, I, (float*)g->w_fc2, M, okt, k.gws, k.gws_bytes, st));
    IA_TRY(dgrad(dy, H, w->w_fc2, w->wt_fc2, I, k.gI, M, IA_EPI_DGELU_COLSUM, s.hpre, I, g->b_fc1, k.ws, k.ws_bytes, st, nullptr, ogrp));
    IA_TRY(wgrad(k.gI, I, s.ln, H, (float*)g->w_fc1, M, okt, k.gws, k.gws_bytes, st));
    IA_TRY(dgrad(k.gI, I, w->w_fc1, w->wt_fc1, H, k.g0, M, IA_EPI_NONE, nullptr, 0, nullptr, nullptr, 0, st, oblk));
    IA_TRY(ia_ln_bwd2_rows(k.g0, nullptr, dy, s.proj, s.mean2, s.rstd2, w->ln2_g, k.g1, nullptr, g->ln2_g, g->ln2_b, g->b_o, M, H, 0.f, 0, 0, olive,
                           k.ws, k.ws_bytes, 1, st));
    IA_TRY(wgrad(k.g1, H, s.ctx, H, (float*)g->w_o, M, okt, k.gws, k.gws_bytes, st));
    IA_TRY(dgrad(k.g1, H, w->w_o, w->wt_o, H, k.g2, M, IA_EPI_NONE, nullptr, 0, nullptr, nullptr, 0, st, oblk));
    IA_TRY(attn_bwd(c, s.qkv, key_mask, s.ctx, k.g2, s.lse, k.delta, k.gqkv, g->b_qkv, k.ws, k.ws_bytes, scale, 0.f, 0, st));
    IA_TRY(ia_gemm_bf16(k.gqkv, 1, 3 * H, s.xn, 1, H, g->w_qkv, 1, H, 3 * H, H, M, IA_EPI_NONE, nullptr, nullptr, 0, nullptr, 1, k.gws, k.gws_bytes, st));
    IA_TRY(dgrad(k.gqkv, 3 * H, w->w_qkv, w->wt_qkv, H, k.g0, M, IA_EPI_NONE, nullptr, 0, nullptr, nullptr, 0, st));
    IA_TRY(ia_ln_bwd(k.g0, k.g1, x, s.mean1, s.rstd1, w->ln1_g, dx, nullptr, g->ln1_g, g->ln1_b, c->dx_colsum_out, M, H, 0.f, 0, 0, k.ws,
                     k.ws_bytes, 1, st));
  }
  return IA_OK;
}
```

item_alignment_amd/csrc/gemm.hip:

```cpp
#include "common.h"
#include <atomic>
#include <cstdlib>
#include <type_traits>

#ifndef IA_GEMM_DBG_HOOKS
#define IA_GEMM_DBG_HOOKS 0
#endif
#define IA_DBG(p) (IA_GEMM_DBG_HOOKS ? (p).dbg : 0)

namespace {

constexpr int BK = 64;
constexpr uint32_t OOB = 0xFFFFFFF0u;

enum { EPI_NONE = 0, EPI_BIAS = 1, EPI_BIAS_GELU = 2, EPI_ADD = 3, EPI_DGELU = 4, EPI_BIAS_ADD = 5, EPI_DGELU_CS = 6, EPI_BIAS_GELU_ACT = 7 };
constexpr int EPI_NONE_LIVE = 8;
constexpr int EPI_ROWS = 16;

struct GemmArgs {
  const bf16* A; const bf16* B; void* C; bf16* C2;
  union {
    const float* bias;
    const uint32_t* live_kt;
  };
// ... 61 lines not shown
#pragma unroll
    for (int r = 0; r < 4; ++r) v[r] += bf2f(a[r]);
  }
  if (EPI == EPI_DGELU || EPI == EPI_DGELU_CS) {
    const bf16x4 a = *reinterpret_cast<const bf16x4*>(p.aux + (size_t)m * p.ldaux + n);
#pragma unroll
    for (int r = 0; r < 4; ++r) v[r] *= bf2f(a[r]);
  }
  if (OUTF32) {
    if (p.splits > 1) {
      *reinterpret_cast<f32x4*>(p.ws + ((size_t)p.split_id * p.M + m) * p.N + n) = v;
      return;
    }
    float* c = reinterpret_cast<float*>(p.C) + (size_t)m * p.ldc + n;
    if (p.accumulate) { const f32x4 o = *reinterpret_cast<const f32x4*>(c); v += o; }
    *reinterpret_cast<f32x4*>(c) = v;
  } else {
    bf16x4 o = {f2bf(v[0]), f2bf(v[1]), f2bf(v[2]), f2bf(v[3])};
    *reinterpret_cast<bf16x4*>(reinterpret_cast<bf16*>(p.C) + (size_t)m * p.ldc + n) = o;
  }
}

template <typename V>
IA_DEV void gstore16(void* ptr, V v) {
  static_assert(sizeof(V) == 16, "16-byte store");
  *reinterpret_cast<V*>(ptr) = v;
}
template <int EPI, bool OUTF32>
constexpr int epi_stores_per_call() { return OUTF32 ? 2 : (EPI == EPI_BIAS_GELU ? 2 : 1); }
template <int EPI>
constexpr int epi_extra_stores() { return EPI == EPI_DGELU_CS ? 2 : 0; }

struct BufIO { __amdgpu_buffer_rsrc_t rsC, rsC2; uint32_t off; };
template <int EPI, bool OUTF32, bool PRE, bool BUF = false>
IA_DEV void epi_store8(const GemmArgs& p, int m, int n, f32x4 lo, f32x4 hi, f32x4 pb0, f32x4 pb1, bf16x8 ax, float (&cs)[8], const BufIO* io = nullptr) {
  float v[8] = {lo[0], lo[1], lo[2], lo[3], hi[0], hi[1], hi[2], hi[3]};
  if (EPI == EPI_BIAS || EPI == EPI_BIAS_GELU || EPI == EPI_BIAS_GELU_ACT || EPI == EPI_BIAS_ADD) {
    const f32x4 b0 = PRE ? pb0 : *reinterpret_cast<const f32x4*>(p.bias + n), b1 = PRE ? pb1 : *reinterpret_cast<const f32x4*>(p.bias + n + 4);
#pragma unroll
    for (int r = 0; r < 4; ++r) { v[r] += b0[r]; v[4 + r] += b1[r]; }
    if (EPI == EPI_BIAS && n < p.qcols) {
#pragma unroll
      for (int r = 0; r < 8; ++r) v[r] *= p.qscale;
    }
  }
  if (EPI == EPI_BIAS_GELU) {
    bf16x8 der;
    {
      constexpr float L2E = 1.4426950408889634f;
      constexpr float C0 = 1.5949398799788077f, C1 = 0.07403000634661838f, C2 = -0.0007007124749191571f;
      constexpr float U_MAX = C1 / (2.f * 0.0007007124749191571f);
      f32x2_t x[4], u[4], t[4], e[4], sg[4], act[4], q[4], d[4];
#pragma unroll
      for (int i = 0; i < 4; ++i) { x[i] = f32x2_t{v[2 * i], v[2 * i + 1]}; u[i] = x[i] * x[i]; }
#pragma unroll
      for (int i = 0; i < 4; ++i) { u[i][0] = __builtin_fminf(u[i][0], U_MAX); u[i][1] = __builtin_fminf(u[i][1], U_MAX); }
#pragma unroll
      for (int i = 0; i < 4; ++i) t[i] = x[i] * ((u[i] * (-C2 * L2E) + (-C1 * L2E)) * u[i] + (-C0 * L2E));
#pragma unroll
      for (int i = 0; i < 4; ++i) e[i] = f32x2_t{__builtin_amdgcn_exp2f(t[i][0]), __builtin_amdgcn_exp2f(t[i][1])};
#pragma unroll
      for (int i = 0; i < 4; ++i) { e[i] = e[i] + 1.0f; q[i] = (u[i] * (5.f * C2) + (3.f * C1)) * u[i] + C0; }
#pragma unroll
      for (int i = 0; i < 4; ++i) sg[i] = f32x2_t{__builtin_amdgcn_rcpf(e[i][0]), __builtin_amdgcn_rcpf(e[i][1])};
#pragma unroll
      for (int i = 0; i < 4; ++i) { act[i] = x[i] * sg[i]; d[i] = (act[i] * (1.0f - sg[i])) * q[i] + sg[i]; }
#pragma unroll
      for (int i = 0; i < 4; ++i) {
        v[2 * i] = act[i][0]; v[2 * i + 1] = act[i][1];
        der[2 * i] = f2bf(d[i][0]); der[2 * i + 1] = f2bf(d[i][1]);
      }
    }
    if (BUF) __builtin_amdgcn_raw_buffer_store_b128(__builtin_bit_cast(u32x4, der), io->rsC2, (int)io->off, 0, 0);
    else gstore16(((IA_DBG(p) & 1024) ? reinterpret_cast<bf16*>(p.C) : p.C2) + (size_t)m * p.ldc + n, der);
  }
  if (EPI == EPI_BIAS_GELU_ACT) {
    constexpr float L2E = 1.4426950408889634f;
    constexpr float C0 = 1.5949398799788077f, C1 = 0.07403000634661838f, C2 = -0.0007007124749191571f;
    constexpr float U_MAX = C1 / (2.f * 0.0007007124749191571f);
    f32x2_t x[4], u[4], t[4], e[4];
#pragma unroll
    for (int i = 0; i < 4; ++i) { x[i] = f32x2_t{v[2 * i], v[2 * i + 1]}; u[i] = x[i] * x[i]; }
#pragma unroll
    for (int i = 0; i < 4; ++i) { u[i][0] = __builtin_fminf(u[i][0], U_MAX); u[i][1] = __builtin_fminf(u[i][1], U_MAX); }
#pragma unroll
    for (int i = 0; i < 4; ++i) t[i] = x[i] * ((u[i] * (-C2 * L2E) + (-C1 * L2E)) * u[i] + (-C0 * L2E));
#pragma unroll
    for (int i = 0; i < 4; ++i) e[i] = f32x2_t{__builtin_amdgcn_exp2f(t[i][0]), __builtin_amdgcn_exp2f(t[i][1])} + 1.0f;
    f32x2_t sg[4], act[4];
#pragma unroll
    for (int i = 0; i < 4; ++i) sg[i] = f32x2_t{__builtin_amdgcn_rcpf(e[i][0]), __builtin_amdgcn_rcpf(e[i][1])};
#pragma unroll
    for (int i = 0; i < 4; ++i) act[i] = x[i] * sg[i];
#pragma unroll
    for (int i = 0; i < 4; ++i) { v[2 * i] = act[i][0]; v[2 * i + 1] = act[i][1]; }
  }
  if (EPI == EPI_ADD || EPI == EPI_BIAS_ADD || EPI == EPI_DGELU || EPI == EPI_DGELU_CS) {
    const bf16x8 a = PRE ? ax : *reinterpret_cast<const bf16x8*>(p.aux + (size_t)m * p.ldaux + n);
#pragma unroll
    for (int r = 0; r < 8; ++r) {
      if (EPI == EPI_DGELU || EPI == EPI_DGELU_CS) v[r] *= bf2f(a[r]);
      else v[r] += bf2f(a[r]);
      if (EPI == EPI_DGELU_CS) cs[r] += v[r];
    }
  }
  if (OUTF32) {
    float* c = p.splits > 1 ? p.ws + ((size_t)p.split_id * p.M + m) * p.N + n : reinterpret_cast<float*>(p.C) + (size_t)m * p.ldc + n;
    f32x4 o0 = {v[0], v[1], v[2], v[3]}, o1 = {v[4], v[5], v[6], v[7]};
    if (p.splits <= 1 && p.accumulate) { o0 += *reinterpret_cast<const f32x4*>(c); o1 += *reinterpret_cast<const f32x4*>(c + 4); }
    gstore16(c, o0);
    gstore16(c + 4, o1);
  } else {
    bf16x8 o;
#pragma unroll
    for (int r = 0; r < 8; ++r) o[r] = f2bf(v[r]);
    if (BUF) __builtin_amdgcn_raw_buffer_store_b128(__builtin_bit_cast(u32x4, o), io->rsC, (int)io->off, 0, 0);
    else gstore16(reinterpret_cast<bf16*>(p.C) + (size_t)m * p.ldc + n, o);
  }
}

IA_DEV int xcd_chunk(int bid, int nwg) {
  const int q = nwg >> 3, r = nwg & 7, xcd = bid & 7, idx = bid >> 3;
  return (xcd < r ? xcd * (q + 1) : r * (q + 1) + (xcd - r) * q) + idx;
}
IA_DEV void tile_of_order(const GemmArgs& p, int t, int& bm, int& bn) {
  const int GM = 8;
  const int group = t / (GM * p.tiles_n);
  const int first_m = group * GM;
  const int gsz = min(p.tiles_m - first_m, GM);
// ... 713 lines not shown
        for (int rg = 0; rg < 4; ++rg) {
          const int chunk = (ni * 32 + (BKS ? rg * 8 + hh * 4 : hh * 16 + rg * 4)) >> 2;
          f32x16& a = acc[mi][NH * 2 + ni];
          const f32x4 v = {a[rg * 4], a[rg * 4 + 1], a[rg * 4 + 2], a[rg * 4 + 3]};
          *reinterpret_cast<f32x4*>(stg + li * 256 + ((chunk ^ (li & 15)) << 4)) = v;
          a[rg * 4] = 0.f; a[rg * 4 + 1] = 0.f; a[rg * 4 + 2] = 0.f; a[rg * 4 + 3] = 0.f;
        }
    };
    stage(0);
#pragma unroll
    for (int mi = 0; mi < 4; ++mi) {
      __builtin_amdgcn_wave_barrier();
      f32x4 lo[4], hi[4];
#pragma unroll
      for (int it = 0; it < 4; ++it) {
        const int row = it * 8 + rrow;
        lo[it] = *reinterpret_cast<const f32x4*>(stg + row * 256 + (((2 * c8) ^ (row & 15)) << 4));
        hi[it] = *reinterpret_cast<const f32x4*>(stg + row * 256 + (((2 * c8 + 1) ^ (row & 15)) << 4));
      }
      asm volatile("s_waitcnt lgkmcnt(0)" : "+v"(lo[0]), "+v"(lo[1]), "+v"(lo[2]), "+v"(lo[3]), "+v"(hi[0]), "+v"(hi[1]), "+v"(hi[2]), "+v"(hi[3]));
      __builtin_amdgcn_wave_barrier();
      if (mi < 3) stage(mi + 1);
#pragma unroll
      for (int it = 0; it < 4; ++it) {
        const int row = it * 8 + rrow;
        const int m = ROWS ? rb.r[mi] + row : m0 + mi * 32 + row, n = n0 + c8 * 8;
        const int c = mi * 4 + it;
        if (PRE) {
          if (HAS_AUX && c + AHEAD < 16) {
            ax[(c + AHEAD) % (AHEAD + 1)] = aux_of(c + AHEAD);
            asm volatile("" ::: "memory");
          }
          io.off = voffC + (uint32_t)(((ROWS ? rb.r[mi] : mi * 32) + it * 8) * p.ldc * 2);
          if (!(IA_DBG(p) & 64)) epi_store8<EPI, OUTF32, true, BUF>(p, m, n, lo[it], hi[it], pb0, pb1, ax[c % (AHEAD + 1)], cs, &io);
        } else {
          if ((!ROWS || rb.r[mi] >= 0) && m < p.M && n < p.N && !(IA_DBG(p) & 64)) epi_store8<EPI, OUTF32, false>(p, m, n, lo[it], hi[it], pb0, pb1, ax[0], cs);
        }
        if (IA_DBG(p) & 64) asm volatile("" : : "v"(lo[it]), "v"(hi[it]));
      }
    }
    if (EPI == EPI_DGELU_CS) {
#pragma unroll
      for (int r = 0; r < 8; ++r) {
        float v = cs[r];
        v += __builtin_bit_cast(float, __builtin_amdgcn_update_dpp(__builtin_bit_cast(int, v), __builtin_bit_cast(int, v), 0x128, 0xF, 0xF, false));
        v = ia_add_xor32(ia_add_xor16(v));
        cs[r] = v;
      }
      int slot = m0 >> 7;
      bool has_slot = true;
      if constexpr (ROWS) {
        if (p.rows_grouped) { slot = rb.r[0] >> 7; has_slot = rb.r[0] >= 0; }
      }
      if (rrow == 0 && n0 + c8 * 8 < p.N && has_slot) {
        float* dst = p.csum_part + (size_t)slot * p.N + n0 + c8 * 8;
        gstore16(dst, f32x4{cs[0], cs[1], cs[2], cs[3]});
        gstore16(dst + 4, f32x4{cs[4], cs[5], cs[6], cs[7]});
      }
    }
  };
  if (full && (HAS_BIAS || HAS_AUX) && !(IA_DBG(p) & 256)) drain(std::true_type{}); else drain(std::false_type{});
}

template <bool AKS, bool BKS, int EPI_, bool OUTF32>
__global__ __launch_bounds__(256) void gemm_kernel(GemmArgs p) {
  constexpr bool LIVE = EPI_ == EPI_NONE_LIVE;
  constexpr bool ROWS = EPI_ >= EPI_ROWS;
  constexpr int EPI = LIVE ? (int)EPI_NONE : (ROWS ? EPI_ - EPI_ROWS : EPI_);
  constexpr bool GUARDABLE = ROWS && EPI == EPI_BIAS;
  static_assert(!LIVE || (AKS && BKS && OUTF32), "live k-tiles: the weight-gradient form only");
  static_assert(!ROWS || (!AKS && !OUTF32 && (EPI == EPI_NONE || EPI == EPI_ADD || EPI == EPI_DGELU_CS ||
                                              (!BKS && (EPI == EPI_BIAS || EPI == EPI_BIAS_GELU || EPI == EPI_BIAS_GELU_ACT || EPI == EPI_BIAS_ADD)))),
                "row remap: the data-gradient forms and the k-contiguous forward forms only");
  extern __shared__ __attribute__((aligned(16))) char smem[];
  const int tid = threadIdx.x, lane0 = tid & 63;
  const int wave = __builtin_amdgcn_readfirstlane(tid >> 6);
  const int wm = wave >> 1, wn = wave & 1;
  const int nk_all = (p.K + BK - 1) / BK;
  [[maybe_unused]] int n_live = 0;
  if constexpr (ROWS) {
    n_live = __builtin_amdgcn_readfirstlane(p.row_blk[0]);
    p.tiles_m = (n_live + 7) >> 3;
    if constexpr (GUARDABLE) {
      if (p.rows_guarded) {
        const int last = n_live > 0 ? __builtin_amdgcn_readfirstlane(p.row_blk[ROW_BLK_HDR + n_live - 1]) : -1;
        p.tiles_m = last >= ((p.M & ~127) >> 5) ? 1 : 0;
      }
    }
  }
  const int total_tiles = p.tiles_m * p.tiles_n;
// ... 136 lines not shown
    run(tile, false, acc, stores_in_flight);
    float ts = 1.f;
    if (bias_pre && BIAS_CT) {
#pragma unroll
      for (int ni = 0; ni < 4; ++ni)
        asm volatile("s_waitcnt vmcnt(0)" : "+v"(bct[ni][0]), "+v"(bct[ni][1]), "+v"(bct[ni][2]), "+v"(bct[ni][3]));
      if (n0_pre < p.qcols) {
        ts = p.qscale;
#pragma unroll
        for (int ni = 0; ni < 4; ++ni)
#pragma unroll
          for (int q = 0; q < 4; ++q) bct[ni][q] *= ts;
      }
    } else if (bias_pre) asm volatile("s_waitcnt vmcnt(0)" : "+v"(pbv[0]), "+v"(pbv[1]), "+v"(pbv[2]), "+v"(pbv[3]));
    int next = ordered ? total_tiles : tile + gridDim.x;
    if (dyn) {
      next = claim_resolve();
      claim_issue();
      if (next < 0) next = total_tiles;
    }
    if (next < total_tiles) run(next, true, acc, false);

    int lane_e = lane0;
    asm volatile("" : "+v"(lane_e));
    int m0 = m0_pre, n0 = n0_pre;
    asm volatile("" : "+s"(m0), "+s"(n0));
    char* stg = smem + 2 * 2 * TILE_BYTES + wave * 2 * STAGE_BYTES;
    bool full_e = full;
    if constexpr (ROWS) {
      const Blk8 bl = tile_blocks<GUARDABLE>(p, bm, n_live);
      RowBlk rb;
#pragma unroll
      for (int mi = 0; mi < 4; ++mi) rb.r[mi] = (wm ? bl.b[4 + mi] : bl.b[mi]) * 32;
      const bool rows_ok = bl.b[7] >= 0 && bl.b[7] * 32 + 32 <= p.M;
      full_e = rows_ok && n0_pre + 128 <= p.N;
      if (!(IA_DBG(p) & 32)) {
        if constexpr (EPI == EPI_NONE) {
          drain_half_plain<BKS, 0, false, true>(p, acc, m0, n0, stg, lane_e, bct, 1.f, rb);
          drain_half_plain<BKS, 1, false, true>(p, acc, m0, n0 + 64, stg, lane_e, bct, 1.f, rb);
        } else if (BIAS_CT && bias_pre) {
          if constexpr (BIAS_CT) {
            drain_half_plain<false, 0, true, true>(p, acc, m0, n0, stg, lane_e, bct, ts, rb);
            drain_half_plain<false, 1, true, true>(p, acc, m0, n0 + 64, stg, lane_e, bct, ts, rb);
          }
        } else {
          drain_half<EPI, OUTF32, BKS, 0, true>(p, acc, m0, n0, stg, lane_e, full_e || (rows_ok && n0 + 64 <= p.N), bias_pre, pbv[0], pbv[1], rb);
          drain_half<EPI, OUTF32, BKS, 1, true>(p, acc, m0, n0 + 64, stg, lane_e, full_e, bias_pre, pbv[2], pbv[3], rb);
        }
      }
    } else
    if (!(IA_DBG(p) & 32)) {
      if constexpr (EPI == EPI_NONE && !OUTF32) {
        drain_half_plain<BKS, 0, false>(p, acc, m0, n0, stg, lane_e, bct);
        drain_half_plain<BKS, 1, false>(p, acc, m0, n0 + 64, stg, lane_e, bct);
      } else if (BIAS_CT && bias_pre) {
        drain_half_plain<false, 0, BIAS_CT>(p, acc, m0, n0, stg, lane_e, bct, ts);
        drain_half_plain<false, 1, BIAS_CT>(p, acc, m0, n0 + 64, stg, lane_e, bct, ts);
      } else {
        drain_half<EPI, OUTF32, BKS, 0>(p, acc, m0, n0, stg, lane_e, full || (m0 + 128 <= p.M && n0 + 64 <= p.N), bias_pre, pbv[0], pbv[1]);
        drain_half<EPI, OUTF32, BKS, 1>(p, acc, m0, n0 + 64, stg, lane_e, full, bias_pre, pbv[2], pbv[3]);
      }
    }
    if (next >= total_tiles) break;
    stores_in_flight = !(IA_DBG(p) & 96) && full_e;
    if (!stores_in_flight) asm volatile("s_waitcnt vmcnt(0)" ::: "memory");
    tile = next;
  }
// ... 278 lines not shown
int g_dynamic = -1;
constexpr int MAX_DEVICES = 16;
uint32_t* g_ctr_base[MAX_DEVICES] = {};
std::atomic<unsigned> g_launch_seq{0};
uint32_t* next_ctr_slot() {
  if (g_dynamic < 0) {
    const char* e = getenv("IA_GEMM_DYNAMIC");
    g_dynamic = e ? atoi(e) : 0;
  }
  if (!g_dynamic) return nullptr;
  int dev = 0;
  if (hipGetDevice(&dev) != hipSuccess || dev < 0 || dev >= MAX_DEVICES) return nullptr;
  uint32_t* base = __atomic_load_n(&g_ctr_base[dev], __ATOMIC_ACQUIRE);
  if (!base) {
    if (hipGetSymbolAddress((void**)&base, HIP_SYMBOL(g_tile_ctr)) != hipSuccess || !base) return nullptr;
    __atomic_store_n(&g_ctr_base[dev], base, __ATOMIC_RELEASE);
  }
  return base + (size_t)(g_launch_seq.fetch_add(1u, std::memory_order_relaxed) % CTR_SLOTS) * CTR_WORDS;
}

__global__ __launch_bounds__(256) void zero_dead_rows_kernel(const int* __restrict__ list, bf16* __restrict__ C, int ldc, int M, int N,
                                                             float* __restrict__ csum_part, int part_rows, int grouped = 0) {
  const int n_live = list[0], n_dead = list[1], nbr = (list[2] + 7) & ~7;
  const int* dead = list + t256w::ROW_BLK_HDR + nbr;
  const int n8 = N >> 3;
  const u32x4 z = {0u, 0u, 0u, 0u};
  for (int d = blockIdx.x; d < n_dead; d += gridDim.x) {
    const int r0 = dead[d] * 32;
    for (int i = threadIdx.x; i < 32 * n8; i += 256) {
      const int r = r0 + i / n8, c = (i % n8) * 8;
      if (r < M) *reinterpret_cast<u32x4*>(C + (size_t)r * ldc + c) = z;
    }
  }
  if (csum_part && grouped) {
    const int ngrp = (M + 127) >> 7;
    for (int d = blockIdx.x; d < n_dead + (part_rows - ngrp); d += gridDim.x) {
      const int g = d < n_dead ? ((dead[d] & 3) ? -1 : dead[d] >> 2) : ngrp + (d - n_dead);
      if (g < 0) continue;
      for (int i = threadIdx.x; i < N; i += 256) csum_part[(size_t)g * N + i] = 0.f;
    }
  } else if (csum_part) {
    const int first = ((n_live + 7) >> 3) * 2;
    const size_t total = part_rows > first ? (size_t)(part_rows - first) * N : 0;
    float* base = csum_part + (size_t)first * N;
    for (size_t i = (size_t)blockIdx.x * 256 + threadIdx.x; i < total; i += (size_t)gridDim.x * 256) base[i] = 0.f;
  }
}

template <bool AKS, bool BKS, int EPI, bool OUTF32>
int launch(GemmArgs a, bool big, hipStream_t st) {
  constexpr int vid = AKS * 1000 + BKS * 100 + EPI * 10 + (OUTF32 ? 1 : 0);
  constexpr bool DROWS = !AKS && !OUTF32 && (EPI == EPI_NONE || EPI == EPI_ADD || EPI == EPI_DGELU_CS ||
                                             (!BKS && (EPI == EPI_BIAS || EPI == EPI_BIAS_GELU || EPI == EPI_BIAS_GELU_ACT || EPI == EPI_BIAS_ADD)));
  constexpr bool WGRAD = AKS && BKS && EPI == EPI_NONE && OUTF32;
  const bool rec = g_prof.on && g_prof.variant == vid && g_prof.n < g_prof.cap && !(WGRAD && a.live_kt) && !(DROWS && a.row_blk);
  if (rec) (void)hipEventRecord(g_prof.ev[2 * g_prof.n], st);
  if (big) {
    a.tiles_m = (a.M + t256w::BM - 1) / t256w::BM; a.tiles_n = (a.N + t256w::BN - 1) / t256w::BN;
    if (a.row_blk && a.rows_guarded) a.tiles_m = 1;
    const int ntile = a.tiles_m * a.tiles_n;
    const int gx = a.splits > 1 ? ntile * a.splits : (ntile < 256 ? ntile : 256);
    a.tile_ctr = (a.splits == 1 && ntile > gx) ? next_ctr_slot() : nullptr;
    void (*kern)(GemmArgs) = t256w::gemm_kernel<AKS, BKS, EPI, OUTF32>;
    static bool attr_set[5] = {false, false, false, false, false};
    int la = 0;
    if constexpr (WGRAD) {
      if (a.live_kt) { kern = t256w::gemm_kernel<true, true, EPI_NONE_LIVE, true>; la = 2; }
// ... 124 lines not shown
extern "C" size_t ia_row_blocks_bytes(int M_rows) {
  if (M_rows <= 0) return 0;
  const size_t nbr = (size_t)(((M_rows + 31) / 32 + 7) & ~7);
  return (t256w::ROW_BLK_HDR + 2 * nbr) * sizeof(int);
}
extern "C" int ia_row_blocks(const uint8_t* row_live, int M_rows, int* list, hipStream_t stream) {
  (void)hipGetLastError();
  if (!row_live || !list || M_rows <= 0 || ((uintptr_t)list & 31)) return IA_ERR_ARG;
  hipLaunchKernelGGL(row_blocks_kernel, dim3(1), dim3(64), 0, stream, row_live, M_rows, (M_rows + 31) / 32, list, 0);
  return ia_check_launch();
}
static int row_blocks_host(const uint8_t* row_live, int M_rows, int* list, int gshift) {
  if (!row_live || !list || M_rows <= 0) return IA_ERR_ARG;
  const int nb = (M_rows + 31) / 32, nbr = (nb + 7) & ~7;
  int* const live = list + t256w::ROW_BLK_HDR;
  int* const dead = live + nbr;
  int n_live = 0;
  for (int t = 0; t < nb; ++t) {
    if (row_block_live(row_live, M_rows, t, gshift)) live[n_live++] = t; else dead[t - n_live] = t;
  }
  for (int i = 0; i < t256w::ROW_BLK_HDR; ++i) list[i] = 0;
  list[0] = n_live; list[1] = nb - n_live; list[2] = nb;
  return IA_OK;
}
extern "C" int ia_row_blocks_host(const uint8_t* row_live, int M_rows, int* list) { return row_blocks_host(row_live, M_rows, list, 0); }
extern "C" size_t ia_row_groups_bytes(int M_rows) { return ia_row_blocks_bytes(M_rows); }
extern "C" int ia_row_groups(const uint8_t* row_live, int M_rows, int* list, hipStream_t stream) {
  (void)hipGetLastError();
  if (!row_live || !list || M_rows <= 0 || ((uintptr_t)list & 31)) return IA_ERR_ARG;
  hipLaunchKernelGGL(row_blocks_kernel, dim3(1), dim3(64), 0, stream, row_live, M_rows, (M_rows + 31) / 32, list, 2);
  return ia_check_launch();
}
extern "C" int ia_row_groups_host(const uint8_t* row_live, int M_rows, int* list) { return row_blocks_host(row_live, M_rows, list, 2); }
int ia_gemm_dgrad_blocks(const void* dY, int ldy, const void* W, int w_kstrided, int ldw, void* dX, int ldx, int M_rows, int N_in, int K_out,
                         int epilogue, const void* aux, int ldaux, void* C2, const int* row_blocks, void* workspace, size_t workspace_bytes,
                         hipStream_t stream) {
  if (epilogue != EPI_NONE && epilogue != EPI_ADD && epilogue != EPI_DGELU_CS) return IA_ERR_UNSUPPORTED;
  return gemm_core(dY, 0, ldy, W, w_kstrided, ldw, dX, 0, ldx, M_rows, N_in, K_out, epilogue, nullptr, aux, ldaux, C2, 0, workspace,
                   workspace_bytes, nullptr, stream, 0, 1.f, nullptr, row_blocks);
}
int ia_gemm_fwd_blocks(const void* X, int ldx, const void* W, int ldw, void* Y, int ldy, int M_rows, int N_out, int K_in, int epilogue,
                       const float* bias, void* C2, int scaled_cols, float col_scale, const int* row_blocks, int fill_dead_rows, hipStream_t stream) {
  if (epilogue != EPI_NONE && epilogue != EPI_BIAS && epilogue != EPI_BIAS_GELU && epilogue != EPI_BIAS_GELU_ACT) return IA_ERR_UNSUPPORTED;
  return gemm_core(X, 0, ldx, W, 0, ldw, Y, 0, ldy, M_rows, N_out, K_in, epilogue, bias, nullptr, 0, C2, 0, nullptr, 0, nullptr, stream, scaled_cols,
                   col_scale, nullptr, row_blocks, fill_dead_rows);
}
int ia_gemm_dgrad_groups(const void* dY, int ldy, const void* W, int w_kstrided, int ldw, void* dX, int ldx, int M_rows, int N_in, int K_out,
                         const void* aux, int ldaux, void* C2, const int* row_groups, void* workspace, size_t workspace_bytes, hipStream_t stream) {
  return gemm_core(dY, 0, ldy, W, w_kstrided, ldw, dX, 0, ldx, M_rows, N_in, K_out, EPI_DGELU_CS, nullptr, aux, ldaux, C2, 0, workspace,
                   workspace_bytes, nullptr, stream, 0, 1.f, nullptr, row_groups, 1, 0, 1);
}
int ia_gemm_fwd_blocks_add(const void* X, int ldx, const void* W, int ldw, void* Y, int ldy, int M_rows, int N_out, int K_in, const float* bias,
                           const void* aux, int ldaux, const int* row_blocks, int fill_dead_rows, hipStream_t stream) {
  return gemm_core(X, 0, ldx, W, 0, ldw, Y, 0, ldy, M_rows, N_out, K_in, EPI_BIAS_ADD, bias, aux, ldaux, nullptr, 0, nullptr, 0, nullptr, stream, 0, 1.f,
                   nullptr, row_blocks, fill_dead_rows);
}
extern "C" int ia_gemm_fwd_rows_add(const void* X, int ldx, const void* W, int ldw, void* Y, int ldy, int M_rows, int N_out, int K_in,
                                    const float* bias, const void* aux, int ldaux, const uint8_t* row_live, int fill_dead_rows, void* workspace,
                                    size_t workspace_bytes, hipStream_t stream) {
  if (!row_live) return ia_gemm_fwd_blocks_add(X, ldx, W, ldw, Y, ldy, M_rows, N_out, K_in, bias, aux, ldaux, nullptr, 0, stream);
  if (M_rows <= 0 || N_out <= 0 || K_in <= 0) return IA_ERR_ARG;
  if (!workspace || workspace_bytes < ia_row_blocks_bytes(M_rows) || ((uintptr_t)workspace & 31)) return IA_ERR_WORKSPACE;
  int rc = ia_row_blocks(row_live, M_rows, (int*)workspace, stream);
  return rc ? rc : ia_gemm_fwd_blocks_add(X, ldx, W, ldw, Y, ldy, M_rows, N_out, K_in, bias, aux, ldaux, (const int*)workspace, fill_dead_rows, stream);
}
extern "C" int ia_gemm_dgrad_groups_rows(const void* dY, int ldy, const void* W, int w_kstrided, int ldw, void* dX, int ldx, int M_rows, int N_in,
// ... 163 lines not shown
  if (view) {
    g.a_view = view->a_view; g.b_view = view->b_view; g.pw = view->pw; g.lca = view->lca; g.lcbk = view->lcbk; g.lcbn = view->lcbn;
    g.groups = groups; g.ga = view->ga; g.gb = view->gb; g.gc = view->gc; g.gbias = view->gbias;
  }
  if (!a_kstrided && (K & 7)) return IA_ERR_ARG;
  g.a_bytes = ab; g.b_bytes = bb;
  g.tiles_m = g.tiles_n = 0;
  { static int dbg = -1; if (dbg < 0) { const char* e = getenv("IA_GEMM_DBG"); dbg = e ? atoi(e) : 0; } g.dbg = dbg; }
  const int nk = (K + BK - 1) / BK;
  Plan pl = make_plan(M, N, K, c_is_f32 != 0, groups);
  g.splits = 1; g.nk_per_split = nk; g.ws = nullptr;
  const bool big = pl.big && !view && !(g.dbg & 128);
  const bool wgrad_form = a_kstrided && b_kstrided && c_is_f32 && epilogue == EPI_NONE;
  g.rsum_out = (wgrad_form && !big) ? (float*)C2 : nullptr;
  g.rsum_ws = nullptr;
  if (c_is_f32 && epilogue == EPI_NONE && pl.splits > 1 && workspace &&
      workspace_bytes >= (size_t)groups * pl.splits * M * (N + (g.rsum_out ? 1 : 0)) * sizeof(float)) {
    g.nk_per_split = (nk + pl.splits - 1) / pl.splits;
    g.splits = (nk + g.nk_per_split - 1) / g.nk_per_split;
    g.ws = (float*)workspace;
    g.rsum_ws = g.ws + (size_t)groups * g.splits * M * N;
  }
  {
    const uint64_t margin = view ? 2 * (uint64_t)(view->pw + 1) : 0, slab = (uint64_t)g.nk_per_split * BK + margin, tile = 256 + margin;
    const uint64_t wa = (a_kstrided ? slab : tile) * (uint64_t)lda * 2 + (a_kstrided ? 0 : (uint64_t)K * 2);
    const uint64_t wb = (b_kstrided ? slab : tile) * (uint64_t)ldb * 2 + (b_kstrided ? 0 : (uint64_t)K * 2);
    if (wa >= 0x7FFFFFF0ull || wb >= 0x7FFFFFF0ull) return IA_ERR_ARG;
  }
  if (a_kstrided && b_kstrided && c_is_f32 && epilogue == EPI_NONE) g.live_kt = (big && g.nk_per_split <= t256w::LIVE_MAX_KTILES) ? live_kt : nullptr;
  const bool fwd_epi = !b_kstrided && (epilogue == EPI_BIAS || epilogue == EPI_BIAS_GELU || epilogue == EPI_BIAS_GELU_ACT || epilogue == EPI_BIAS_ADD);
  g.row_blk = nullptr; g.rows_fill = rows_fill; g.fill_m = M; g.rows_guarded = tail_of ? 1 : 0;
  if (!a_kstrided && !c_is_f32 && (epilogue == EPI_NONE || epilogue == EPI_ADD || epilogue == EPI_DGELU_CS || fwd_epi))
    g.row_blk = (row_blocks && big && !g.dbg && !(N & 7) && dgrad_rows_fit(M, lda, ldc, aux ? ldaux : 0)) ? row_blocks : nullptr;
  g.rows_grouped = (g.row_blk && epilogue == EPI_DGELU_CS && rows_grouped) ? 1 : 0;
  if (g.row_blk && fwd_epi && qcols > 0 && (M & 127) && !tail_of) {
    const int Mb = M & ~127;
    int rc = gemm_core(A, 0, lda, B, 0, ldb, C, 0, ldc, M, N, K, epilogue, bias, nullptr, 0, nullptr, 0, nullptr, 0, nullptr, stream, qcols, qscale, nullptr,
                       row_blocks, 0, 1);
    if (rc) return rc;
    g.a_bytes = ((uint64_t)(Mb - 1) * lda + K) * 2;
    g.M = Mb;
  }
  const bool needs_bias = epilogue == EPI_BIAS || epilogue == EPI_BIAS_GELU || epilogue == EPI_BIAS_GELU_ACT || epilogue == EPI_BIAS_ADD;
  const bool needs_aux = epilogue == EPI_ADD || epilogue == EPI_DGELU || epilogue == EPI_BIAS_ADD || epilogue == EPI_DGELU_CS;
  if (needs_bias && !bias) return IA_ERR_ARG;
  if (needs_aux && (!aux || (ldaux & 3))) return IA_ERR_ARG;
  if (epilogue == EPI_BIAS_GELU && !C2) return IA_ERR_ARG;

  if (!a_kstrided && !b_kstrided && !c_is_f32) {
    switch (epilogue) {
      case EPI_NONE: return launch<false, false, EPI_NONE, false>(g, big, stream);
      case EPI_BIAS: return launch<false, false, EPI_BIAS, false>(g, big, stream);
      case EPI_BIAS_GELU: return launch<false, false, EPI_BIAS_GELU, false>(g, big, stream);
      case EPI_BIAS_GELU_ACT: return launch<false, false, EPI_BIAS_GELU_ACT, false>(g, big, stream);
      case EPI_BIAS_ADD: return launch<false, false, EPI_BIAS_ADD, false>(g, big, stream);
      case EPI_ADD: return launch<false, false, EPI_ADD, false>(g, big, stream);
      case EPI_DGELU: return launch<false, false, EPI_DGELU, false>(g, big, stream);
      case EPI_DGELU_CS: return launch_dgelu_colsum<false>(g, big, (float*)C2, workspace, workspace_bytes, stream);
    }
  } else if (!a_kstrided && b_kstrided && !c_is_f32) {
    switch (epilogue) {
      case EPI_NONE: return launch<false, true, EPI_NONE, false>(g, big, stream);
      case EPI_ADD: return launch<false, true, EPI_ADD, false>(g, big, stream);
      case EPI_DGELU: return launch<false, true, EPI_DGELU, false>(g, big, stream);
      case EPI_DGELU_CS: return launch_dgelu_colsum<true>(g, big, (float*)C2, workspace, workspace_bytes, stream);
    }
  } else if (a_kstrided && b_kstrided && c_is_f32) {
// ... 71 lines not shown
```

item_alignment_amd/models/functional.py:

```python
import ctypes as C

import torch

from .. import _lib
from .._lib import LayerCfg, LayerGrads, LayerWeights, check, ptr, stream_ptr

BF16, F32 = torch.bfloat16, torch.float32
_step_seed = [0x1234567]


def set_step_seed(seed):
    _step_seed[0] = int(seed) & 0xFFFFFFFF


def step_seed():
    return _step_seed[0]


def _need_gpu(t, what):
    if not t.is_cuda:
        raise _lib.ItemAlignError(f"{what} is on {t.device}: the MI355X engine has no CPU path (move the model and batch to cuda)")


_notify_hooks = []
# ... 102 lines not shown
    check(lib.ia_row_blocks(p, M, p + o_blk, stream_ptr()), "ia_row_blocks")
    check(lib.ia_ktile_mask(p, M, p + o_kt, stream_ptr()), "ia_ktile_mask")
    check(lib.ia_row_groups(p, M, p + o_grp, stream_ptr()), "ia_row_groups")
    got = (buf, p, p + o_blk, p + o_kt, p + o_grp)
    if key_mask is None and not torch.cuda.is_current_stream_capturing():
        while len(_cls_row_lists) >= _CLS_ROW_LISTS_KEPT:
            _cls_row_lists.pop(next(iter(_cls_row_lists)))
        _cls_row_lists[key] = got
    return got


class EncoderStackFn(torch.autograd.Function):

    @staticmethod
    def forward(ctx, x, anchor, stack, key_mask, B, L, keep, cu_seqlens=None):
        lib = _lib.load()
        _need_gpu(x, "hidden states")
        ctx.set_materialize_grads(False)
        n = len(stack.layers)
        training = stack.training and keep
        seed = step_seed()
        cfgs = [stack.layer_cfg(i, B, L, training, seed) for i in range(n)]
        if cu_seqlens is not None:
            for c in cfgs:
                c.cu_seqlens, c.total_tokens = cu_seqlens.data_ptr(), x.shape[0]
        ctx.cu_seqlens = cu_seqlens
        outs, cur = [], x.contiguous()
        inputs = [cur]
        mp = ptr(key_mask)
        ctx.row_lists = None
        flag = cfgs[0].masked_rows_dead
        if key_mask is not None and cu_seqlens is None and not cfgs[0].pre_ln and ((flag & 1 and keep) or (flag & 3) == 3):
            M = cur.shape[0]
            lb = (lib.ia_row_blocks_bytes(M) + 255) & ~255
            lists = torch.empty(lb + lib.ia_ktile_mask_bytes(M), device=x.device, dtype=torch.uint8)
            check(lib.ia_row_blocks(mp, M, lists.data_ptr(), stream_ptr()), "ia_row_blocks")
            if keep:
                check(lib.ia_ktile_mask(mp, M, lists.data_ptr() + lb, stream_ptr()), "ia_ktile_mask")
            for c in cfgs:
                c.row_blocks, c.live_ktiles = lists.data_ptr(), (lists.data_ptr() + lb) if keep else None
            ctx.row_lists = lists
        ctx.out_lists = None
        if stack.__dict__.get("_out_rows_cls") and cu_seqlens is None:
            ctx.out_lists = cls_row_lists(B, L, x.device, key_mask)
            c = cfgs[-1]
            c.out_row_live, c.out_row_blocks, c.out_live_ktiles, c.out_row_groups = ctx.out_lists[1:]
        if keep:
            stash_bytes = lib.ia_layer_stash_bytes(C.byref(cfgs[0]))
            stash = [torch.empty(stash_bytes, device=x.device, dtype=torch.uint8) for _ in range(n)]
            for i in range(n):
                y = torch.empty_like(cur)
                check(lib.ia_layer_fwd(C.byref(cfgs[i]), C.byref(stack.weights(i)), cur.data_ptr(), mp, y.data_ptr(),
                                       stash[i].data_ptr(), stream_ptr()), f"ia_layer_fwd[{i}]")
                outs.append(y)
                cur = y
                inputs.append(cur)
        else:
            stash_bytes, stash = 0, None
            sbytes = lib.ia_layer_infer_scratch_bytes(C.byref(cfgs[0]))
            scratch = torch.empty(sbytes, device=x.device, dtype=torch.uint8)
            for i in range(n):
                y = torch.empty_like(cur)
                check(lib.ia_layer_fwd_infer(C.byref(cfgs[i]), C.byref(stack.weights(i)), cur.data_ptr(), mp, y.data_ptr(), scratch.data_ptr(),
                                             sbytes, stream_ptr()), f"ia_layer_fwd_infer[{i}]")
                outs.append(y)
                cur = y
            inputs = None
        ctx.stack, ctx.cfgs, ctx.stash, ctx.stash_bytes = stack, cfgs, stash, stash_bytes
        ctx.inputs, ctx.key_mask = inputs, key_mask
        if keep:
            _pending_uses[id(stack)] = _pending_uses.get(id(stack), 0) + 1
        return tuple(outs)

    @staticmethod
    def backward(ctx, *grads):
        lib = _lib.load()
        stack, cfgs, n = ctx.stack, ctx.cfgs, len(ctx.cfgs)
        scratch_bytes = lib.ia_layer_bwd_scratch_bytes(C.byref(cfgs[0]))
        scratch = torch.empty(scratch_bytes, device=ctx.stash[0].device, dtype=torch.uint8)
# ... 654 lines not shown
```

Baseline: 692.4.

## Limit last-layer attention to CLS query rows and pack live row groups for dgrad

Adds a q_rows limit so that, in the final encoder layer where only the CLS output is consumed, the attention forward and backward kernels compute just the first query rows and zero the rest. It also adds a packed row-group list, built by a single-wave kernel that sorts 128-row groups by how many of their 32-row blocks are live, and a dgrad GEMM path that uses it for the DGELU-colsum epilogue. Both aim to skip GEMM and attention work on masked or unused rows. The cost is extra list-building kernels, more bookkeeping in the attention kernels, and a correctness risk if any consumer reads the zeroed rows.

Result: faster. 703.0, median of 6 (+1.5%).

```diff
diff --git a/include/itemalign.h b/include/itemalign.h
--- a/include/itemalign.h
+++ b/include/itemalign.h
@@ -66,6 +66,14 @@
                               int K_out, const void* aux, int ldaux, void* C2, const uint8_t* row_live, void* workspace,
                               size_t workspace_bytes, ia_stream_t stream);
 int ia_debug_out_rows(int on);
+size_t ia_row_groups_packed_bytes(int M_rows);
+size_t ia_row_groups_packed_offset(int M_rows);
+int ia_row_groups_packed(const uint8_t* row_live, int M_rows, int* list, ia_stream_t stream);
+int ia_row_groups_packed_host(const uint8_t* row_live, int M_rows, int* list);
+int ia_gemm_dgrad_packed(const void* dY, int ldy, const void* W, int w_kstrided, int ldw, void* dX, int ldx, int M_rows, int N_in, int K_out,
+                         const void* aux, int ldaux, void* C2, const int* packed_list, void* workspace, size_t workspace_bytes,
+                         ia_stream_t stream);
+int ia_debug_q_rows(int on);
 
 int ia_prof_begin(int variant, int max_launches);
 int ia_prof_end(double* total_ms, double* total_flops, int* launches);
@@ -115,6 +123,12 @@
                         const void* d_out, int ld_o, const float* lse2, float* delta, void* dq, void* dk, void* dv, int ld_dqkv, float* dbias,
                         void* workspace, size_t workspace_bytes, int B, int nh, int L, float scale, float drop_p, uint32_t seed,
                         ia_stream_t stream);
+int ia_attn_fwd_q_rows(int flags, const void* q, const void* k, const void* v, int ld_qkv, const uint8_t* key_mask, void* out, int ld_o,
+                       float* lse2, int B, int nh, int L, float scale, float drop_p, uint32_t seed, int q_rows, ia_stream_t stream);
+int ia_attn_bwd_bias_q_rows(int flags, const void* q, const void* k, const void* v, int ld_qkv, const uint8_t* key_mask, const void* out,
+                            const void* d_out, int ld_o, const float* lse2, float* delta, void* dq, void* dk, void* dv, int ld_dqkv,
+                            float* dbias, void* workspace, size_t workspace_bytes, int B, int nh, int L, float scale, float drop_p,
+                            uint32_t seed, int q_rows, ia_stream_t stream);
 
 int ia_attn_fwd_x(const void* q, int ld_q, const void* k, const void* v, int ld_kv, const uint8_t* key_mask, void* out, int ld_o,
                   float* lse2, int B, int nh, int Lq, int Lk, float scale, float drop_p, uint32_t seed, ia_stream_t stream);
@@ -343,6 +357,7 @@
   uint32_t layer_id;
   const int* cu_seqlens;
   int total_tokens;
+  int out_q_rows;
   float* dx_colsum_out;
   int dy_colsum_done;
   int masked_rows_dead;
diff --git a/item_alignment_amd/_lib.py b/item_alignment_amd/_lib.py
--- a/item_alignment_amd/_lib.py
+++ b/item_alignment_amd/_lib.py
@@ -21,6 +21,7 @@
 class LayerCfg(C.Structure):
     _fields_ = [("B", i32), ("L", i32), ("H", i32), ("I", i32), ("nh", i32), ("pre_ln", i32), ("eps", f32),
                 ("hidden_drop", f32), ("attn_drop", f32), ("seed", u32), ("layer_id", u32), ("cu_seqlens", vp), ("total_tokens", i32),
+                ("out_q_rows", i32),
                 ("dx_colsum_out", vp), ("dy_colsum_done", i32), ("masked_rows_dead", i32),
                 ("row_blocks", vp), ("live_ktiles", vp),
                 ("out_row_live", vp), ("out_row_blocks", vp), ("out_live_ktiles", vp), ("out_row_groups", vp)]
@@ -55,6 +56,12 @@
     "ia_row_groups_host": (i32, [vp, i32, vp]),
     "ia_gemm_dgrad_groups_rows": (i32, [vp, i32, vp, i32, i32, vp, i32, i32, i32, i32, vp, i32, vp, vp, vp, sz, vp]),
     "ia_debug_out_rows": (i32, [i32]),
+    "ia_row_groups_packed_bytes": (sz, [i32]),
+    "ia_row_groups_packed_offset": (sz, [i32]),
+    "ia_row_groups_packed": (i32, [vp, i32, vp, vp]),
+    "ia_row_groups_packed_host": (i32, [vp, i32, vp]),
+    "ia_gemm_dgrad_packed": (i32, [vp, i32, vp, i32, i32, vp, i32, i32, i32, i32, vp, i32, vp, vp, vp, sz, vp]),
+    "ia_debug_q_rows": (i32, [i32]),
     "ia_prof_begin": (i32, [i32, i32]),
     "ia_prof_end": (i32, [C.POINTER(C.c_double), C.POINTER(C.c_double), C.POINTER(i32)]),
     "ia_prof_bytes": (C.c_double, []),
@@ -75,6 +82,8 @@
     "ia_attn_fwd_ps": (i32, [vp, vp, vp, i32, vp, vp, i32, vp, i32, i32, i32, f32, f32, u32, vp]),
     "ia_attn_bwd_bias_ps": (i32, [vp, vp, vp, i32, vp, vp, vp, i32, vp, vp, vp, vp, vp, i32, vp, vp, sz, i32, i32, i32, f32, f32, u32, vp]),
     "ia_attn_bwd_bias_ex": (i32, [i32, vp, vp, vp, i32, vp, vp, vp, i32, vp, vp, vp, vp, vp, i32, vp, vp, sz, i32, i32, i32, f32, f32, u32, vp]),
+    "ia_attn_fwd_q_rows": (i32, [i32, vp, vp, vp, i32, vp, vp, i32, vp, i32, i32, i32, f32, f32, u32, i32, vp]),
+    "ia_attn_bwd_bias_q_rows": (i32, [i32, vp, vp, vp, i32, vp, vp, vp, i32, vp, vp, vp, vp, vp, i32, vp, vp, sz, i32, i32, i32, f32, f32, u32, i32, vp]),
     "ia_gemm_bf16_qscale": (i32, [vp, i32, vp, i32, vp, i32, i32, i32, i32, vp, i32, f32, vp]),
     "ia_attn_fwd_x": (i32, [vp, i32, vp, vp, i32, vp, vp, i32, vp, i32, i32, i32, i32, f32, f32, u32, vp]),
     "ia_attn_bwd_x": (i32, [vp, i32, vp, vp, i32, vp, vp, vp, i32, vp, vp, vp, i32, vp, vp, i32, i32, i32, i32, i32, f32, f32, u32, vp]),
diff --git a/item_alignment_amd/csrc/attention.hip b/item_alignment_amd/csrc/attention.hip
--- a/item_alignment_amd/csrc/attention.hip
+++ b/item_alignment_amd/csrc/attention.hip
@@ -30,6 +30,7 @@
   float* cs_part;
   int exact_delta;
   int dead_queries;
+  int q_lim;
 };
 
 IA_DEV void attn_block_coords(const AttnArgs& p, int nt, int& tile, int& h, int& b) {
@@ -149,6 +150,12 @@
 }
 IA_DEV void zero_cs_row(float* cs_out, int lane) {
   if (lane < 16) *reinterpret_cast<f32x4*>(cs_out + lane * 4) = f32x4{0.f, 0.f, 0.f, 0.f};
+}
+IA_DEV void zero_unread_rows(const AttnArgs& p, size_t qbase, int b, int h, int q0, int nq, int Lq, int lane) {
+  const int c = lane & 7;
+  for (int r = lane >> 3; r < nq && q0 + r < Lq; r += 8)
+    *reinterpret_cast<u32x4*>(p.out + (qbase + q0 + r) * p.ld_o + h * 64 + c * 8) = u32x4{0u, 0u, 0u, 0u};
+  if (p.lse2 && lane < nq && q0 + lane < Lq) p.lse2[((size_t)b * p.nh + h) * p.Lq + q0 + lane] = 0.f;
 }
 
 namespace fwd3 {
@@ -293,7 +300,12 @@
     if (tile * ROWS >= Lq) return;
   }
   const int q0 = tile * ROWS + wave * 32 * QB;
-  const bool active = q0 < Lq;
+  const bool unread = p.q_lim > 0 && q0 >= p.q_lim;
+  if (unread) {
+    if (q0 < Lq) zero_unread_rows(p, qbase, b, h, q0, 32 * QB, Lq, lane);
+    if (tile * ROWS >= p.q_lim) return;
+  }
+  const bool active = q0 < Lq && !unread;
   const uint32_t win = (uint32_t)(((size_t)(L - 1) * p.ld_kv + 64) * 2);
   const __amdgpu_buffer_rsrc_t rsK = ia_rsrc(p.k + rowbase * p.ld_kv + h * 64, win);
   const __amdgpu_buffer_rsrc_t rsV = ia_rsrc(p.v + rowbase * p.ld_kv + h * 64, win);
@@ -596,6 +608,10 @@
     if (t128 + 1 < nkt_all) any |= s_valid[t128 + 1][0] | s_valid[t128 + 1][1];
     work = active && __builtin_amdgcn_readfirstlane(mine) != 0u;
     if (__builtin_amdgcn_readfirstlane(any) == 0u) nkt = 1;
+  }
+  if (p.q_lim > 0) {
+    work = work && q0 < p.q_lim;
+    if (tile * 128 >= p.q_lim) nkt = 1;
   }
   nkt = __builtin_amdgcn_readfirstlane(nkt);
   ragged = __builtin_amdgcn_readfirstlane(ragged);
@@ -975,6 +991,12 @@
     const int live = __builtin_amdgcn_readfirstlane(last < 0 ? 1 : (last >> 6) + 1);
     if (live < nqt) nqt = live;
   }
+  int qend = Lq;
+  if (p.q_lim > 0 && p.q_lim < Lq) {
+    qend = p.q_lim;
+    const int live = (qend + 63) >> 6;
+    if (live < nqt) nqt = live;
+  }
   if (nqt > 1) stage_tile(S1{}, 1);
   f32x16 dk0 = zero16(), dk1 = zero16(), dv0 = zero16(), dv1 = zero16();
 
@@ -1077,7 +1099,7 @@
       else asm volatile("s_waitcnt vmcnt(0)" ::: "memory");
       prescale(((decltype(SLOT_T)::value + 1) % 3) * KV_STAGE);
     }
-    if (qt * 64 + 32 < Lq) sub_tile(std::integral_constant<int, 1>{});
+    if (qt * 64 + 32 < qend) sub_tile(std::integral_constant<int, 1>{});
   };
   {
     int qt = 0;
@@ -1257,6 +1279,7 @@
   bool any_bad = false;
   uint32_t pc = 0u, ush = 0u;
   const int G = cnt * nb;
+  const uint32_t qlim_bits = p.q_lim > 0 ? (1u << ((p.q_lim + 31) >> 5)) - 1u : 0xFFFFFFFFu;
   int cj = 0;
   Cur prev = cons;
   int pcj = 0;
@@ -1301,7 +1324,7 @@
           dk0 = zero16(); dk1 = zero16(); dv0 = zero16(); dv1 = zero16();
           csq = f32x4{0.f, 0.f, 0.f, 0.f};
         }
-        if (mine && (!p.dead_queries || ((vbits >> blk) & 1u))) {
+        if (mine && ((qlim_bits >> blk) & 1u) && (!p.dead_queries || ((vbits >> blk) & 1u))) {
           const uint32_t so = (uint32_t)(slot * SLOT);
           f32x16 s, dp;
           const float* const sL = reinterpret_cast<const float*>(smem + RING_OFF + slot * SLOT + SL_LSE) + 4 * hh;
@@ -1387,7 +1410,7 @@
         const uint32_t xr = xrb + ((g - 1) & 1) * XT, xr2 = xr ^ 16u;
         s16x4 lo[8], hi[8];
         f32x4 acc = {0.f, 0.f, 0.f, 0.f};
-        if (!p.dead_queries || ((vbits >> pcj) & 1u)) {
+        if (((qlim_bits >> pcj) & 1u) && (!p.dead_queries || ((vbits >> pcj) & 1u))) {
 #pragma unroll
         for (int k = 0; k < 8; ++k) { lo[k] = tr_read<0>(xr + k * 2 * XT); hi[k] = tr_read<16 * XP>(xr2 + k * 2 * XT); }
 #define IA_DQ_STEP(k, n)                                                                                   \
@@ -1521,8 +1544,11 @@
 struct Packed { const int* cu; int total; };
 struct BiasOut { float* dbias; void* workspace; size_t workspace_bytes; };
 
+int q_lim_of(int q_rows, bool packed, int Lq) { return (q_rows > 0 && !packed && q_rows < Lq) ? q_rows : 0; }
+
 int attn_fwd_impl(int flags, const void* q, int ld_q, const void* k, const void* v, int ld_kv, const uint8_t* key_mask, const Packed* pk, void* out,
-                  int ld_o, float* lse2, int B, int nh, int Lq, int Lk, float scale, float drop_p, uint32_t seed, hipStream_t stream) {
+                  int ld_o, float* lse2, int B, int nh, int Lq, int Lk, float scale, float drop_p, uint32_t seed, hipStream_t stream,
+                  int q_rows = 0) {
   (void)hipGetLastError();
   if (!q || !k || !v || !out || (pk && (!pk->cu || pk->total <= 0))) return IA_ERR_ARG;
   AttnArgs a{};
@@ -1531,6 +1557,7 @@
   a.q = (const bf16*)q; a.k = (const bf16*)k; a.v = (const bf16*)v; a.out = (bf16*)out; a.mask = key_mask; a.lse2 = lse2;
   a.cu = pk ? pk->cu : nullptr;
   a.q_prescaled = (flags & IA_ATTN_Q_PRESCALED) ? 1 : 0;
+  a.q_lim = q_lim_of(q_rows, pk != nullptr, Lq);
   if (a.thr16) launch_fwd<true>(a, stream);
   else launch_fwd<false>(a, stream);
   return ia_check_launch();
@@ -1538,7 +1565,8 @@
 
 int attn_bwd_impl(int flags, const void* q, int ld_q, const void* k, const void* v, int ld_kv, const uint8_t* key_mask, const Packed* pk,
                   const void* out, const void* d_out, int ld_o, const float* lse2, float* delta, void* dq, int ld_dq, void* dk, void* dv, int ld_dkv,
-                  const BiasOut* bias, int B, int nh, int Lq, int Lk, float scale, float drop_p, uint32_t seed, hipStream_t stream) {
+                  const BiasOut* bias, int B, int nh, int Lq, int Lk, float scale, float drop_p, uint32_t seed, hipStream_t stream,
+                  int q_rows = 0) {
   (void)hipGetLastError();
   if (!q || !k || !v || !out || !d_out || !lse2 || !delta || !dq || !dk || !dv) return IA_ERR_ARG;
   if ((pk && (!pk->cu || pk->total <= 0)) || (bias && !bias->dbias)) return IA_ERR_ARG;
@@ -1554,6 +1582,7 @@
   a.q_prescaled = (flags & IA_ATTN_Q_PRESCALED) ? 1 : 0;
   a.dead_queries = ((flags & IA_ATTN_MASKED_ROWS_DEAD) && key_mask) ? 1 : 0;
   a.exact_delta = exact_delta_on() ? 1 : 0;
+  a.q_lim = q_lim_of(q_rows, pk != nullptr, Lq);
   if (a.thr16) launch_bwd<true>(a, stream);
   else launch_bwd<false>(a, stream);
   rc = ia_check_launch();
@@ -1609,6 +1638,20 @@
   return attn_bwd_impl(flags, q, ld_qkv, k, v, ld_qkv, key_mask, nullptr, out, d_out, ld_o, lse2, delta, dq, ld_dqkv, dk, dv, ld_dqkv, &bias, B, nh, L, L,
                        scale, drop_p, seed, stream);
 }
+extern "C" int ia_attn_fwd_q_rows(int flags, const void* q, const void* k, const void* v, int ld_qkv, const uint8_t* key_mask, void* out, int ld_o,
+                                  float* lse2, int B, int nh, int L, float scale, float drop_p, uint32_t seed, int q_rows, hipStream_t stream) {
+  if (flags & ~IA_ATTN_Q_PRESCALED) return IA_ERR_ARG;
+  return attn_fwd_impl(flags, q, ld_qkv, k, v, ld_qkv, key_mask, nullptr, out, ld_o, lse2, B, nh, L, L, scale, drop_p, seed, stream, q_rows);
+}
+extern "C" int ia_attn_bwd_bias_q_rows(int flags, const void* q, const void* k, const void* v, int ld_qkv, const uint8_t* key_mask, const void* out,
+                                       const void* d_out, int ld_o, const float* lse2, float* delta, void* dq, void* dk, void* dv, int ld_dqkv,
+                                       float* dbias, void* workspace, size_t workspace_bytes, int B, int nh, int L, float scale, float drop_p,
+                                       uint32_t seed, int q_rows, hipStream_t stream) {
+  if (flags & ~(IA_ATTN_Q_PRESCALED | IA_ATTN_MASKED_ROWS_DEAD)) return IA_ERR_ARG;
+  const BiasOut bias{dbias, workspace, workspace_bytes};
+  return attn_bwd_impl(flags, q, ld_qkv, k, v, ld_qkv, key_mask, nullptr, out, d_out, ld_o, lse2, delta, dq, ld_dqkv, dk, dv, ld_dqkv, &bias, B, nh, L, L,
+                       scale, drop_p, seed, stream, q_rows);
+}
 extern "C" int ia_attn_bwd_bias(const void* q, const void* k, const void* v, int ld_qkv, const uint8_t* key_mask, const void* out,
                                 const void* d_out, int ld_o, const float* lse2, float* delta, void* dq, void* dk, void* dv, int ld_dqkv,
                                 float* dbias, void* workspace, size_t workspace_bytes, int B, int nh, int L, float scale, float drop_p,
diff --git a/item_alignment_amd/csrc/engine.hip b/item_alignment_amd/csrc/engine.hip
--- a/item_alignment_amd/csrc/engine.hip
+++ b/item_alignment_amd/csrc/engine.hip
@@ -65,6 +65,7 @@
 
 struct Scratch {
   char* g0; char* g1; char* g2; char* gI; char* gqkv; float* delta; char* ws; size_t ws_bytes; char* gws; size_t gws_bytes; uint32_t* live_kt; int* row_blk;
+  int* pack_blk;
   uint32_t* out_kt; int* out_blk; int* out_grp;
   size_t bytes;
 };
@@ -86,6 +87,7 @@
   s.gws = a.take(s.gws_bytes);
   s.live_kt = (uint32_t*)a.take(ia_ktile_mask_bytes((int)M));
   s.row_blk = (int*)a.take(ia_row_blocks_bytes((int)M));
+  s.pack_blk = (int*)a.take(ia_row_groups_packed_bytes((int)M));
   s.out_kt = (uint32_t*)a.take(ia_ktile_mask_bytes((int)M));
   s.out_blk = (int*)a.take(ia_row_blocks_bytes((int)M));
   s.out_grp = (int*)a.take(ia_row_groups_bytes((int)M));
@@ -102,13 +104,17 @@
 int g_fwd_rows = 1;
 int g_out_rows = 1;
 const uint8_t* out_live(const ia_layer_cfg* c) { return (c->out_row_live && !c->cu_seqlens && g_out_rows) ? c->out_row_live : nullptr; }
+int g_q_rows = 1;
+int out_q_rows(const ia_layer_cfg* c) { return (out_live(c) && c->out_q_rows > 0 && g_q_rows) ? c->out_q_rows : 0; }
 
 #define IA_TRY(expr) do { int rc_ = (expr); if (rc_) return rc_; } while (0)
 
 int dgrad(const void* dy, int k_out, const void* w, const void* wt, int n_in, void* dx, int M, int epilogue, const void* aux, int ldaux, void* c2,
-          void* ws, size_t ws_bytes, ia_stream_t st, const int* row_blk = nullptr, const int* row_grp = nullptr) {
+          void* ws, size_t ws_bytes, ia_stream_t st, const int* row_blk = nullptr, const int* row_grp = nullptr, const int* row_pack = nullptr) {
   if (row_grp && epilogue == IA_EPI_DGELU_COLSUM)
     return ia_gemm_dgrad_groups(dy, k_out, wt ? wt : w, wt ? 0 : 1, wt ? k_out : n_in, dx, n_in, M, n_in, k_out, aux, ldaux, c2, row_grp, ws, ws_bytes, st);
+  if (row_pack && epilogue == IA_EPI_DGELU_COLSUM)
+    return ia_gemm_dgrad_packed(dy, k_out, wt ? wt : w, wt ? 0 : 1, wt ? k_out : n_in, dx, n_in, M, n_in, k_out, aux, ldaux, c2, row_pack, ws, ws_bytes, st);
   if (row_blk)
     return ia_gemm_dgrad_blocks(dy, k_out, wt ? wt : w, wt ? 0 : 1, wt ? k_out : n_in, dx, n_in, M, n_in, k_out, epilogue, aux, ldaux, c2, row_blk,
                                 ws, ws_bytes, st);
@@ -140,7 +146,8 @@
   if (c->cu_seqlens)
     return (ps ? ia_attn_fwd_varlen_ps : ia_attn_fwd_varlen)(qkv, qkv + (size_t)H * 2, qkv + (size_t)2 * H * 2, 3 * H, c->cu_seqlens, c->total_tokens, ctx, H, lse, c->B, c->nh,
                               c->L, scale, drop, seed, st);
-  return (ps ? ia_attn_fwd_ps : ia_attn_fwd)(qkv, qkv + (size_t)H * 2, qkv + (size_t)2 * H * 2, 3 * H, key_mask, ctx, H, lse, c->B, c->nh, c->L, scale, drop, seed, st);
+  return ia_attn_fwd_q_rows(ps ? IA_ATTN_Q_PRESCALED : 0, qkv, qkv + (size_t)H * 2, qkv + (size_t)2 * H * 2, 3 * H, key_mask, ctx, H, lse, c->B, c->nh,
+                            c->L, scale, drop, seed, out_q_rows(c), st);
 }
 
 int attn_bwd(const ia_layer_cfg* c, const char* qkv, const uint8_t* key_mask, const char* ctx, const char* dctx, const float* lse, float* delta,
@@ -153,8 +160,9 @@
     return rc ? rc : ia_colsum(gqkv, 3 * H, (int)rows_of(c), 3 * H, db_qkv, 1, ws, ws_bytes, st);
   }
   const int flags = (ps ? IA_ATTN_Q_PRESCALED : 0) | ((c->masked_rows_dead & 1) ? IA_ATTN_MASKED_ROWS_DEAD : 0);
-  return ia_attn_bwd_bias_ex(flags, qkv, qkv + (size_t)H * 2, qkv + (size_t)2 * H * 2, 3 * H, key_mask, ctx, dctx, H, lse, delta, gqkv,
-                             gqkv + (size_t)H * 2, gqkv + (size_t)2 * H * 2, 3 * H, db_qkv, ws, ws_bytes, c->B, c->nh, c->L, scale, drop, seed, st);
+  return ia_attn_bwd_bias_q_rows(flags, qkv, qkv + (size_t)H * 2, qkv + (size_t)2 * H * 2, 3 * H, key_mask, ctx, dctx, H, lse, delta, gqkv,
+                                 gqkv + (size_t)H * 2, gqkv + (size_t)2 * H * 2, 3 * H, db_qkv, ws, ws_bytes, c->B, c->nh, c->L, scale, drop, seed,
+                                 out_q_rows(c), st);
 }
 
 int layer_forward(const ia_layer_cfg* c, const ia_layer_weights* w, const void* x, const uint8_t* key_mask, void* y, const FwdBufs& s,
@@ -224,6 +232,12 @@
 extern "C" int ia_debug_out_rows(int on) {
   const int was = g_out_rows;
   g_out_rows = on ? 1 : 0;
+  return was;
+}
+
+extern "C" int ia_debug_q_rows(int on) {
+  const int was = g_q_rows;
+  g_q_rows = on ? 1 : 0;
   return was;
 }
 
@@ -305,6 +319,11 @@
     const int* const row_blk = (live && g_dgrad_rows) ? (c->row_blocks ? c->row_blocks : k.row_blk) : nullptr;
     if (live && !c->live_ktiles) IA_TRY(ia_ktile_mask(live, M, k.live_kt, st));
     if (row_blk && !c->row_blocks) IA_TRY(ia_row_blocks(live, M, k.row_blk, st));
+    const int* row_pack = nullptr;
+    if (row_blk && (size_t)M <= (size_t)128 * 4096) {
+      if (c->row_blocks && (c->masked_rows_dead & 4)) row_pack = (const int*)((const char*)c->row_blocks + ia_row_groups_packed_offset(M));
+      else { IA_TRY(ia_row_groups_packed(live, M, k.pack_blk, st)); row_pack = k.pack_blk; }
+    }
     const uint8_t* const live2 = olive ? olive : live;
     const uint32_t* const kt2 = olive ? okt : live_kt;
     const int* const blk2 = olive ? oblk : row_blk;
@@ -312,7 +331,7 @@
                            c->hidden_drop, c->seed, c->layer_id * 4u + 1u, live2, k.ws, k.ws_bytes, 1, st));
     const char* d_ffn = drop ? k.g1 : k.g0;
     IA_TRY(wgrad(d_ffn, H, s.hact, I, (float*)g->w_fc2, M, kt2, k.gws, k.gws_bytes, st));
-    IA_TRY(dgrad(d_ffn, H, w->w_fc2, w->wt_fc2, I, k.gI, M, IA_EPI_DGELU_COLSUM, s.hpre, I, g->b_fc1, k.ws, k.ws_bytes, st, nullptr, ogrp));
+    IA_TRY(dgrad(d_ffn, H, w->w_fc2, w->wt_fc2, I, k.gI, M, IA_EPI_DGELU_COLSUM, s.hpre, I, g->b_fc1, k.ws, k.ws_bytes, st, nullptr, ogrp, row_pack));
     IA_TRY(wgrad(k.gI, I, s.ln, H, (float*)g->w_fc1, M, kt2, k.gws, k.gws_bytes, st));
     IA_TRY(dgrad(k.gI, I, w->w_fc1, w->wt_fc1, H, k.g2, M, IA_EPI_NONE, nullptr, 0, nullptr, nullptr, 0, st, blk2));
     char* dz1buf = dx2 ? (char*)dx2 : k.g0;
diff --git a/item_alignment_amd/csrc/gemm.hip b/item_alignment_amd/csrc/gemm.hip
--- a/item_alignment_amd/csrc/gemm.hip
+++ b/item_alignment_amd/csrc/gemm.hip
@@ -117,7 +117,7 @@
 constexpr int epi_extra_stores() { return EPI == EPI_DGELU_CS ? 2 : 0; }
 
 struct BufIO { __amdgpu_buffer_rsrc_t rsC, rsC2; uint32_t off; };
-template <int EPI, bool OUTF32, bool PRE, bool BUF = false>
+template <int EPI, bool OUTF32, bool PRE, bool BUF = false, bool PIN = false>
 IA_DEV void epi_store8(const GemmArgs& p, int m, int n, f32x4 lo, f32x4 hi, f32x4 pb0, f32x4 pb1, bf16x8 ax, float (&cs)[8], const BufIO* io = nullptr) {
   float v[8] = {lo[0], lo[1], lo[2], lo[3], hi[0], hi[1], hi[2], hi[3]};
   if (EPI == EPI_BIAS || EPI == EPI_BIAS_GELU || EPI == EPI_BIAS_GELU_ACT || EPI == EPI_BIAS_ADD) {
@@ -180,6 +180,21 @@
 #pragma unroll
     for (int i = 0; i < 4; ++i) { v[2 * i] = act[i][0]; v[2 * i + 1] = act[i][1]; }
   }
+  if constexpr (EPI == EPI_DGELU_CS && PIN) {
+    const bf16x8 a = PRE ? ax : *reinterpret_cast<const bf16x8*>(p.aux + (size_t)m * p.ldaux + n);
+    if (PRE) {
+#pragma clang fp contract(off)
+#pragma unroll
+      for (int r = 0; r < 8; ++r) { v[r] *= bf2f(a[r]); cs[r] += v[r]; }
+    } else {
+#pragma unroll
+      for (int r = 0; r < 8; ++r) {
+        const float x = v[r], y = bf2f(a[r]);
+        v[r] = x * y;
+        cs[r] = __builtin_fmaf(x, y, cs[r]);
+      }
+    }
+  } else
   if (EPI == EPI_ADD || EPI == EPI_BIAS_ADD || EPI == EPI_DGELU || EPI == EPI_DGELU_CS) {
     const bf16x8 a = PRE ? ax : *reinterpret_cast<const bf16x8*>(p.aux + (size_t)m * p.ldaux + n);
 #pragma unroll
@@ -959,14 +974,34 @@
             asm volatile("" ::: "memory");
           }
           io.off = voffC + (uint32_t)(((ROWS ? rb.r[mi] : mi * 32) + it * 8) * p.ldc * 2);
-          if (!(IA_DBG(p) & 64)) epi_store8<EPI, OUTF32, true, BUF>(p, m, n, lo[it], hi[it], pb0, pb1, ax[c % (AHEAD + 1)], cs, &io);
+          if (!(IA_DBG(p) & 64)) epi_store8<EPI, OUTF32, true, BUF, ROWS>(p, m, n, lo[it], hi[it], pb0, pb1, ax[c % (AHEAD + 1)], cs, &io);
         } else {
-          if ((!ROWS || rb.r[mi] >= 0) && m < p.M && n < p.N && !(IA_DBG(p) & 64)) epi_store8<EPI, OUTF32, false>(p, m, n, lo[it], hi[it], pb0, pb1, ax[0], cs);
+          if ((!ROWS || rb.r[mi] >= 0) && m < p.M && n < p.N && !(IA_DBG(p) & 64)) epi_store8<EPI, OUTF32, false, false, ROWS>(p, m, n, lo[it], hi[it], pb0, pb1, ax[0], cs);
         }
         if (IA_DBG(p) & 64) asm volatile("" : : "v"(lo[it]), "v"(hi[it]));
       }
+      if constexpr (ROWS && EPI == EPI_DGELU_CS) {
+        if (p.rows_grouped == 2 && rb.r[mi] >= 0 && (mi == 3 || rb.r[mi < 3 ? mi + 1 : 3] < 0 || (rb.r[mi < 3 ? mi + 1 : 3] >> 7) != (rb.r[mi] >> 7))) {
+#pragma unroll
+          for (int r = 0; r < 8; ++r) {
+            float v = cs[r];
+            v += __builtin_bit_cast(float, __builtin_amdgcn_update_dpp(__builtin_bit_cast(int, v), __builtin_bit_cast(int, v), 0x128, 0xF, 0xF, false));
+            cs[r] = ia_add_xor32(ia_add_xor16(v));
+          }
+          if (rrow == 0 && n0 + c8 * 8 < p.N) {
+            float* dst = p.csum_part + (size_t)(rb.r[mi] >> 7) * p.N + n0 + c8 * 8;
+            gstore16(dst, f32x4{cs[0], cs[1], cs[2], cs[3]});
+            gstore16(dst + 4, f32x4{cs[4], cs[5], cs[6], cs[7]});
+          }
+#pragma unroll
+          for (int r = 0; r < 8; ++r) cs[r] = 0.f;
+        }
+      }
     }
     if (EPI == EPI_DGELU_CS) {
+      bool packed = false;
+      if constexpr (ROWS) packed = p.rows_grouped == 2;
+      if (!packed) {
 #pragma unroll
       for (int r = 0; r < 8; ++r) {
         float v = cs[r];
@@ -983,6 +1018,7 @@
         float* dst = p.csum_part + (size_t)slot * p.N + n0 + c8 * 8;
         gstore16(dst, f32x4{cs[0], cs[1], cs[2], cs[3]});
         gstore16(dst + 4, f32x4{cs[4], cs[5], cs[6], cs[7]});
+      }
       }
     }
   };
@@ -1185,7 +1221,14 @@
       RowBlk rb;
 #pragma unroll
       for (int mi = 0; mi < 4; ++mi) rb.r[mi] = (wm ? bl.b[4 + mi] : bl.b[mi]) * 32;
-      const bool rows_ok = bl.b[7] >= 0 && bl.b[7] * 32 + 32 <= p.M;
+      bool rows_ok = bl.b[7] >= 0 && bl.b[7] * 32 + 32 <= p.M;
+      if constexpr (EPI == EPI_DGELU_CS) {
+        if (p.rows_grouped == 2) {
+          rows_ok = rb.r[0] >= 0;
+#pragma unroll
+          for (int mi = 0; mi < 4; ++mi) rows_ok = rows_ok && (rb.r[mi] < 0 || (rb.r[mi] | 127) < p.M);
+        }
+      }
       full_e = rows_ok && n0_pre + 128 <= p.N;
       if (!(IA_DBG(p) & 32)) {
         if constexpr (EPI == EPI_NONE) {
@@ -1530,7 +1573,10 @@
       if (r < M) *reinterpret_cast<u32x4*>(C + (size_t)r * ldc + c) = z;
     }
   }
-  if (csum_part && grouped) {
+  if (csum_part && grouped == 2) {
+    const size_t total = (size_t)part_rows * N;
+    for (size_t i = (size_t)blockIdx.x * 256 + threadIdx.x; i < total; i += (size_t)gridDim.x * 256) csum_part[i] = 0.f;
+  } else if (csum_part && grouped) {
     const int ngrp = (M + 127) >> 7;
     for (int d = blockIdx.x; d < n_dead + (part_rows - ngrp); d += gridDim.x) {
       const int g = d < n_dead ? ((dead[d] & 3) ? -1 : dead[d] >> 2) : ngrp + (d - n_dead);
@@ -1721,6 +1767,132 @@
   return ia_check_launch();
 }
 extern "C" int ia_row_groups_host(const uint8_t* row_live, int M_rows, int* list) { return row_blocks_host(row_live, M_rows, list, 2); }
+struct PackCounts { int n4, n3, n2, n1; };
+static __host__ __device__ inline int pack_left1(const PackCounts& n) { return n.n1 > n.n3 ? n.n1 - n.n3 : 0; }
+static __host__ __device__ inline int pack_take2(const PackCounts& n) { const int l = pack_left1(n); return (n.n2 & 1) ? (l < 2 ? l : 2) : 0; }
+static __host__ __device__ inline int pack_rows(const PackCounts& n) {
+  return n.n4 + n.n3 + ((n.n2 + 1) >> 1) + ((pack_left1(n) - pack_take2(n) + 3) >> 2);
+}
+static __host__ __device__ inline void pack_place(const PackCounts& n, int c, int r, int& slot, int& pad) {
+  const int base2 = n.n4 + n.n3, base1 = base2 + ((n.n2 + 1) >> 1), take2 = pack_take2(n);
+  pad = 0;
+  if (c == 4) slot = 4 * r;
+  else if (c == 3) { slot = 4 * (n.n4 + r); pad = r < n.n1 ? 0 : 1; }
+  else if (c == 2) { slot = 4 * (base2 + (r >> 1)) + 2 * (r & 1); pad = ((n.n2 & 1) && r == n.n2 - 1 && take2 == 0) ? 2 : 0; }
+  else if (r < n.n3) slot = 4 * (n.n4 + r) + 3;
+  else if (r - n.n3 < take2) { slot = 4 * (base2 + (n.n2 >> 1)) + 2 + (r - n.n3); pad = (r - n.n3 == take2 - 1) ? 2 - take2 : 0; }
+  else {
+    const int q = r - n.n3 - take2;
+    slot = 4 * base1 + q;
+    pad = r == n.n1 - 1 ? 3 - (q & 3) : 0;
+  }
+}
+namespace {
+constexpr int PACK_MAX_GROUPS = 64 * 64;
+__global__ __launch_bounds__(64) void row_groups_packed_kernel(const uint8_t* __restrict__ row_live, int M, int nb, int* __restrict__ out) {
+  const int nbr = (nb + 7) & ~7, ngrp = (nb + 3) >> 2;
+  int* const live = out + t256w::ROW_BLK_HDR;
+  int* const dead = live + nbr;
+  const int lane = threadIdx.x;
+  const uint64_t lt = (1ull << lane) - 1ull;
+  uint64_t f[4] = {0, 0, 0, 0};
+  for (int i = 0; i * 64 < ngrp; ++i) {
+    const int g = i * 64 + lane;
+#pragma unroll
+    for (int j = 0; j < 4; ++j)
+      if (g < ngrp && 4 * g + j < nb && row_block_live(row_live, M, 4 * g + j)) f[j] |= 1ull << i;
+  }
+  auto cls = [&](int i) { return (int)((f[0] >> i) & 1ull) + (int)((f[1] >> i) & 1ull) + (int)((f[2] >> i) & 1ull) + (int)((f[3] >> i) & 1ull); };
+  const int cut = (M & 127) ? ngrp - 1 : -1;
+  int cnt[5] = {0, 0, 0, 0, 0}, cut_rows = 0;
+  for (int i = 0; i * 64 < ngrp; ++i) {
+    const bool is_cut = i * 64 + lane == cut;
+    const int c = is_cut ? 0 : cls(i);
+#pragma unroll
+    for (int k = 1; k <= 4; ++k) cnt[k] += __popcll(__ballot(c == k));
+    cut_rows += __ballot(is_cut && cls(i) > 0) ? 1 : 0;
+  }
+  const PackCounts n{cnt[4], cnt[3], cnt[2], cnt[1]};
+  int rank[5] = {0, 0, 0, 0, 0}, dbase = 0;
+  for (int i = 0; i * 64 < ngrp; ++i) {
+    const int g = i * 64 + lane, c_all = cls(i), c = g == cut ? 0 : c_all;
+    int nblk = g < ngrp ? nb - 4 * g : 0;
+    nblk = nblk > 4 ? 4 : nblk;
+    const int nd = nblk - c_all;
+    int r = 0, dpos = dbase;
+#pragma unroll
+    for (int k = 1; k <= 4; ++k) {
+      const uint64_t b = __ballot(c == k), d = __ballot(nd >= k);
+      if (c == k) r = rank[k] + __popcll(b & lt);
+      rank[k] += __popcll(b);
+      dpos += __popcll(d & lt);
+      dbase += __popcll(d);
+    }
+    if (g < ngrp) {
+      if (c_all > 0) {
+        int slot, pad;
+        if (g == cut) { slot = 4 * pack_rows(n); pad = 4 - c_all; }
+        else pack_place(n, c, r, slot, pad);
+#pragma unroll
+        for (int j = 0; j < 4; ++j)
+          if ((f[j] >> i) & 1ull) live[slot++] = 4 * g + j;
+        for (int k = 0; k < pad; ++k) live[slot++] = -1;
+      }
+#pragma unroll
+      for (int j = 0; j < 4; ++j)
+        if (j < nblk && !((f[j] >> i) & 1ull)) dead[dpos++] = 4 * g + j;
+    }
+  }
+  if (lane < t256w::ROW_BLK_HDR) out[lane] = lane == 0 ? 4 * (pack_rows(n) + cut_rows) : (lane == 1 ? dbase : (lane == 2 ? nb : 0));
+}
+}
+extern "C" size_t ia_row_groups_packed_bytes(int M_rows) { return ia_row_blocks_bytes(M_rows); }
+extern "C" size_t ia_row_groups_packed_offset(int M_rows) { return al256(ia_row_blocks_bytes(M_rows)); }
+extern "C" int ia_row_groups_packed(const uint8_t* row_live, int M_rows, int* list, hipStream_t stream) {
+  (void)hipGetLastError();
+  if (!row_live || !list || M_rows <= 0 || ((uintptr_t)list & 31)) return IA_ERR_ARG;
+  if ((M_rows + 127) / 128 > PACK_MAX_GROUPS) return IA_ERR_UNSUPPORTED;
+  hipLaunchKernelGGL(row_groups_packed_kernel, dim3(1), dim3(64), 0, stream, row_live, M_rows, (M_rows + 31) / 32, list);
+  return ia_check_launch();
+}
+extern "C" int ia_row_groups_packed_host(const uint8_t* row_live, int M_rows, int* list) {
+  if (!row_live || !list || M_rows <= 0) return IA_ERR_ARG;
+  if ((M_rows + 127) / 128 > PACK_MAX_GROUPS) return IA_ERR_UNSUPPORTED;
+  const int nb = (M_rows + 31) / 32, nbr = (nb + 7) & ~7, ngrp = (nb + 3) >> 2;
+  int* const live = list + t256w::ROW_BLK_HDR;
+  int* const dead = live + nbr;
+  PackCounts n{0, 0, 0, 0};
+  auto cls = [&](int g) {
+    int c = 0;
+    for (int j = 0; j < 4 && 4 * g + j < nb; ++j) c += row_block_live(row_live, M_rows, 4 * g + j) ? 1 : 0;
+    return c;
+  };
+  const int cut = (M_rows & 127) ? ngrp - 1 : -1;
+  for (int g = 0; g < ngrp; ++g) {
+    const int c = g == cut ? 0 : cls(g);
+    if (c == 4) ++n.n4; else if (c == 3) ++n.n3; else if (c == 2) ++n.n2; else if (c == 1) ++n.n1;
+  }
+  int rank[5] = {0, 0, 0, 0, 0}, n_dead = 0, cut_rows = 0;
+  for (int g = 0; g < ngrp; ++g) {
+    const int c = cls(g);
+    int slot = 0, pad = 0;
+    if (g == cut && c > 0) { slot = 4 * pack_rows(n); pad = 4 - c; cut_rows = 1; }
+    else if (c > 0) pack_place(n, c, rank[c]++, slot, pad);
+    for (int j = 0; j < 4 && 4 * g + j < nb; ++j) {
+      if (row_block_live(row_live, M_rows, 4 * g + j)) live[slot++] = 4 * g + j; else dead[n_dead++] = 4 * g + j;
+    }
+    for (int k = 0; k < pad; ++k) live[slot++] = -1;
+  }
+  for (int i = 0; i < t256w::ROW_BLK_HDR; ++i) list[i] = 0;
+  list[0] = 4 * (pack_rows(n) + cut_rows); list[1] = n_dead; list[2] = nb;
+  return IA_OK;
+}
+extern "C" int ia_gemm_dgrad_packed(const void* dY, int ldy, const void* W, int w_kstrided, int ldw, void* dX, int ldx, int M_rows, int N_in, int K_out,
+                                    const void* aux, int ldaux, void* C2, const int* packed_list, void* workspace, size_t workspace_bytes,
+                                    hipStream_t stream) {
+  return gemm_core(dY, 0, ldy, W, w_kstrided, ldw, dX, 0, ldx, M_rows, N_in, K_out, EPI_DGELU_CS, nullptr, aux, ldaux, C2, 0, workspace,
+                   workspace_bytes, nullptr, stream, 0, 1.f, nullptr, packed_list, 1, 0, packed_list ? 2 : 0);
+}
 int ia_gemm_dgrad_blocks(const void* dY, int ldy, const void* W, int w_kstrided, int ldw, void* dX, int ldx, int M_rows, int N_in, int K_out,
                          int epilogue, const void* aux, int ldaux, void* C2, const int* row_blocks, void* workspace, size_t workspace_bytes,
                          hipStream_t stream) {
@@ -1950,7 +2122,7 @@
   g.row_blk = nullptr; g.rows_fill = rows_fill; g.fill_m = M; g.rows_guarded = tail_of ? 1 : 0;
   if (!a_kstrided && !c_is_f32 && (epilogue == EPI_NONE || epilogue == EPI_ADD || epilogue == EPI_DGELU_CS || fwd_epi))
     g.row_blk = (row_blocks && big && !g.dbg && !(N & 7) && dgrad_rows_fit(M, lda, ldc, aux ? ldaux : 0)) ? row_blocks : nullptr;
-  g.rows_grouped = (g.row_blk && epilogue == EPI_DGELU_CS && rows_grouped) ? 1 : 0;
+  g.rows_grouped = (g.row_blk && epilogue == EPI_DGELU_CS && rows_grouped) ? rows_grouped : 0;
   if (g.row_blk && fwd_epi && qcols > 0 && (M & 127) && !tail_of) {
     const int Mb = M & ~127;
     int rc = gemm_core(A, 0, lda, B, 0, ldb, C, 0, ldc, M, N, K, epilogue, bias, nullptr, 0, nullptr, 0, nullptr, 0, nullptr, stream, qcols, qscale, nullptr,
diff --git a/item_alignment_amd/models/functional.py b/item_alignment_amd/models/functional.py
--- a/item_alignment_amd/models/functional.py
+++ b/item_alignment_amd/models/functional.py
@@ -158,19 +158,25 @@
         flag = cfgs[0].masked_rows_dead
         if key_mask is not None and cu_seqlens is None and not cfgs[0].pre_ln and ((flag & 1 and keep) or (flag & 3) == 3):
             M = cur.shape[0]
-            lb = (lib.ia_row_blocks_bytes(M) + 255) & ~255
-            lists = torch.empty(lb + lib.ia_ktile_mask_bytes(M), device=x.device, dtype=torch.uint8)
+            lb = lib.ia_row_groups_packed_offset(M)
+            packed = keep and M <= 128 * 4096
+            lists = torch.empty(2 * lb + lib.ia_ktile_mask_bytes(M), device=x.device, dtype=torch.uint8)
             check(lib.ia_row_blocks(mp, M, lists.data_ptr(), stream_ptr()), "ia_row_blocks")
+            if packed:
+                check(lib.ia_row_groups_packed(mp, M, lists.data_ptr() + lb, stream_ptr()), "ia_row_groups_packed")
             if keep:
-                check(lib.ia_ktile_mask(mp, M, lists.data_ptr() + lb, stream_ptr()), "ia_ktile_mask")
+                check(lib.ia_ktile_mask(mp, M, lists.data_ptr() + 2 * lb, stream_ptr()), "ia_ktile_mask")
             for c in cfgs:
-                c.row_blocks, c.live_ktiles = lists.data_ptr(), (lists.data_ptr() + lb) if keep else None
+                c.row_blocks, c.live_ktiles = lists.data_ptr(), (lists.data_ptr() + 2 * lb) if keep else None
+                if packed:
+                    c.masked_rows_dead |= 4
             ctx.row_lists = lists
         ctx.out_lists = None
         if stack.__dict__.get("_out_rows_cls") and cu_seqlens is None:
             ctx.out_lists = cls_row_lists(B, L, x.device, key_mask)
             c = cfgs[-1]
             c.out_row_live, c.out_row_blocks, c.out_live_ktiles, c.out_row_groups = ctx.out_lists[1:]
+            c.out_q_rows = 1
         if keep:
             stash_bytes = lib.ia_layer_stash_bytes(C.byref(cfgs[0]))
             stash = [torch.empty(stash_bytes, device=x.device, dtype=torch.uint8) for _ in range(n)]
```
